# tohinz/multiple-objects-gan

Hardware: AMD Instinct MI355X
Metric: images/sec per G+D train step, 256x256 coco-attngan (higher is better)
Workload: dtype f32

## Files before the change

include/mogan_hip.h:

```cpp
#ifndef MOGAN_HIP_H
#define MOGAN_HIP_H

#include <stddef.h>
#include <stdint.h>

#ifdef __cplusplus
extern "C" {
#endif

typedef struct ihipStream_t* hipStream_t;

#define MOGAN_ERR_SHAPE (-1)
#define MOGAN_ERR_LAUNCH (-2)
#define MOGAN_ERR_WS (-3)

#define MOGAN_ACT_NONE 0
#define MOGAN_ACT_RELU 1
#define MOGAN_ACT_LRELU 2
#define MOGAN_ACT_GLU 3
#define MOGAN_ACT_TANH 4
#define MOGAN_ACT_SIGMOID 5

int mogan_abi_version(void);
int mogan_gemm_set_split_target(int blocks);
int mogan_stream_set_split_target(hipStream_t stream, int blocks);

int mogan_gemm_tune_set(int mode, int M, int N, int K, int nz, int cfg, int split);
int mogan_gemm_tune_clear(void);

int mogan_reserve_streams(int n);

int mogan_gemm_debug_force(int cfg, int split);
int mogan_gemm_group_min_tiles(int tiles);
int mogan_mfma_form(void);

int mogan_prof_enable(int on);
int mogan_prof_collect(double* out, int max_rows);
int mogan_prof_dump(const char* path);

int mogan_conv2d_out_dims(int Hs, int Ws, int KH, int KW, int stride, int ph, int pw, int up, int* OH, int* OW);
int mogan_conv2d_fwd(const float* x, const float* w, float* y, int B, int Cin, int Hs, int Ws, int Cout, int KH,
                     int KW, int stride, int ph, int pw, int up, void* ws, size_t ws_bytes, hipStream_t stream);
int mogan_logits_head_fwd(const float* x, const float* w, const float* bias, float* p, int B, int K, int Cout,
                          hipStream_t stream);
int mogan_logits_head_bwd(const float* dp, const float* p, const float* x, const float* w, float* dx, float* dw, float* db,
                          int B, int K, int Cout, int accumulate, hipStream_t stream);
int mogan_conv2d_lrelu_fwd(const float* x, const float* w, float* z, int B, int Cin, int Hs, int Ws, int Cout, int KH, int KW,
                           int stride, int ph, int pw, float slope, void* ws, size_t ws_bytes, hipStream_t stream);
int mogan_conv2d_affine_fwd(const float* x, const float* w, const float* scale, const float* shift, float* y, int B,
                            int Cin, int Hs, int Ws, int Cout, int KH, int KW, int stride, int ph, int pw, int relu,
                            void* ws, size_t ws_bytes, hipStream_t stream);
int mogan_affine_relu_bwd_out(const float* y, const float* dy, const float* scale, float* dx, int B, int C, int HW,
                              hipStream_t stream);
typedef struct MoganConvFwdArgs {
    const float* x; long long x_bstride; const float* w; const float* scale; const float* shift;
    float* y; long long y_bstride; float* y2; long long y2_bstride; int msplit;
    int B, Cin, Hs, Ws, Cout, KH, KW, stride, ph, pw, relu;
} MoganConvFwdArgs;
typedef struct MoganConvDgradArgs {
    const float* dy; long long dy_bstride; const float* w; float* dx; long long dx_bstride;
    const float* relu_of; long long relu_bstride; int accumulate;
    int B, Cin, Hs, Ws, Cout, KH, KW, stride, ph, pw;
} MoganConvDgradArgs;
int mogan_conv2d_affine_fwd_group(int n, const MoganConvFwdArgs* args, void* ws, size_t ws_bytes, hipStream_t stream);
int mogan_conv2d_dgrad_group(int n, const MoganConvDgradArgs* args, void* ws, size_t ws_bytes, hipStream_t stream);
int mogan_conv2d_affine_fwd_ex(const float* x, long long x_bstride, const float* w, const float* scale, const float* shift,
                               float* y, long long y_bstride, float* y2, long long y2_bstride, int msplit, int B, int Cin,
                               int Hs, int Ws, int Cout, int KH, int KW, int stride, int ph, int pw, int relu, void* ws,
                               size_t ws_bytes, hipStream_t stream);
int mogan_conv2d_fwd_ex(const float* x, long long x_bstride, const float* w, float* y, long long y_bstride,
                        const float* relu_of, long long relu_bstride, int accumulate, int B, int Cin, int Hs, int Ws,
                        int Cout, int KH, int KW, int stride, int ph, int pw, void* ws, size_t ws_bytes, hipStream_t stream);
int mogan_conv2d_dgrad_ex(const float* dy, long long dy_bstride, const float* w, float* dx, long long dx_bstride,
                          const float* relu_of, long long relu_bstride, int accumulate, int B, int Cin, int Hs, int Ws,
                          int Cout, int KH, int KW, int stride, int ph, int pw, void* ws, size_t ws_bytes,
                          hipStream_t stream);
int mogan_conv2d_dgrad(const float* dy, const float* w, float* dx, int B, int Cin, int Hs, int Ws, int Cout, int KH,
                       int KW, int stride, int ph, int pw, int up, void* ws, size_t ws_bytes, hipStream_t stream);
size_t mogan_wino_prep_bytes(int B, int Cin, int Hs, int Ws, int Cout, int KH, int KW, int stride, int ph, int pw, int up, int dgrad);
int mogan_wino_prep_group(int n, const float* const* w, void* const* prep, const int* Cout, const int* Cin, const int* dgrad,
                          hipStream_t stream);
size_t mogan_conv_prep_bytes(int B, int Cin, int Hs, int Ws, int Cout, int KH, int KW, int stride, int ph, int pw, int up, int dgrad);
int mogan_conv_prep_group(int n, const float* const* w, void* const* prep, const int* Cout, const int* Cin, const int* KH,
                          const int* dgrad, hipStream_t stream);
int mogan_conv2d_fwd_wp(const float* x, const float* w, const void* wprep, float* y, int B, int Cin, int Hs, int Ws, int Cout, int KH,
                        int KW, int stride, int ph, int pw, int up, void* ws, size_t ws_bytes, hipStream_t stream);
int mogan_conv2d_dgrad_wp(const float* dy, const float* w, const void* wprep, float* dx, int B, int Cin, int Hs, int Ws, int Cout,
                          int KH, int KW, int stride, int ph, int pw, int up, void* ws, size_t ws_bytes, hipStream_t stream);
int mogan_conv2d_wgrad(const float* dy, const float* x, float* dw, int B, int Cin, int Hs, int Ws, int Cout, int KH,
                       int KW, int stride, int ph, int pw, int up, int accumulate, void* ws, size_t ws_bytes,
                       hipStream_t stream);

int mogan_pk_conv_eligible(int B, int Cin, int Hs, int Ws, int Cout, int KH, int KW, int stride, int ph, int pw, int dgrad);
size_t mogan_pk_weight_bytes(int Cout, int Cin, int KH, int KW, int stride, int dgrad);
int mogan_pk_weight_pack(const float* w, void* wpk, int Cout, int Cin, int KH, int KW, int stride, int ph, int pw, int dgrad,
                         hipStream_t stream);
int mogan_pk_weight_pack_both(const float* w, void* wpk_fwd, void* wpk_dgrad, int Cout, int Cin, int KH, int KW, int stride, int ph,
                              int pw, hipStream_t stream);
int mogan_pk_adam_pack_both(float* p, float* g, float* m, float* v, float* ema, void* wpk_fwd, void* wpk_dgrad, int Cout, int Cin,
                            int KH, int KW, int stride, int ph, int pw, float lr, float beta1, float beta2, float eps, int step,
                            const float* dev_state, int eps_mode, float grad_scale, float ema_decay, int zero_g,
                            hipStream_t stream);
int mogan_conv2d_fwd_pk(const float* x, const void* wpk, float* y, int B, int Cin, int Hs, int Ws, int Cout, int KH, int KW,
                        int stride, int ph, int pw, void* ws, size_t ws_bytes, hipStream_t stream);
int mogan_conv2d_dgrad_pk(const float* dy, const void* wpk, float* dx, int B, int Cin, int Hs, int Ws, int Cout, int KH, int KW,
                          int stride, int ph, int pw, void* ws, size_t ws_bytes, hipStream_t stream);
int mogan_pk_debug_force(int take_all, int cfg, int split);
int mogan_pk_wgrad_eligible(int B, int Cin, int Hs, int Ws, int Cout, int KH, int KW, int stride, int ph, int pw, size_t ws_bytes);
int mogan_conv2d_wgrad_pk(const float* dy, const float* x, float* dw, int B, int Cin, int Hs, int Ws, int Cout, int KH, int KW,
                          int stride, int ph, int pw, int accumulate, void* ws, size_t ws_bytes, hipStream_t stream);

size_t mogan_pk_panel_bytes(int B, int C, int HW);
int mogan_deep_block_eligible(int B, int Cin, int Hs, int Ws, int Cout, int KH, int KW, int stride, int ph, int pw, int act,
                              int groups);
int mogan_deep_conv_bn_act_fwd(const float* x, const void* xpanel, const void* wpk, const float* gamma, const float* beta,
                               float* rmean, float* rvar, float* y, float* stats, float* z, void* zpanel, int B, int Cin, int Hs,
                               int Ws, int Cout, int KH, int KW, int stride, int ph, int pw, float eps, float momentum, int act,
                               float slope, int groups, void* ws, size_t ws_bytes, hipStream_t stream);
int mogan_deep_conv_bn_act_bwd(const float* dz, const float* y, const float* stats, const float* gamma, const float* beta,
                               const void* wpk_dgrad, float* dy, float* dgamma, float* dbeta, int accumulate, float* dx, int B,
                               int Cin, int Hs, int Ws, int Cout, int KH, int KW, int stride, int ph, int pw, int act, float slope,
                               int groups, void* ws, size_t ws_bytes, hipStream_t stream);

typedef struct MoganPkArgs {
    const void* wpk; const void* panel; float* raw;
    int B, M;
    int Cp, CGp, cg0;
    int PH, PW, outH, outW;
    int KH, KW, stride, ph, pw, dgrad;
    int nsplit;
} MoganPkArgs;
#define MOGAN_TAIL_MAXSRC 3
typedef struct MoganTailArgs {
    const float* src[MOGAN_TAIL_MAXSRC]; long long src_bs[MOGAN_TAIL_MAXSRC]; long long src_slab[MOGAN_TAIL_MAXSRC];
    int src_nsplit[MOGAN_TAIL_MAXSRC]; int nsrc;
    const float* add; long long add_bs;
    const float* mask; long long mask_bs;
    const float* scale; const float* shift;
    int relu, box;
    float* dst; long long dst_bs;
    void* panel; int CGp, cg0;
    int B, n, H, W;
} MoganTailArgs;
int mogan_pk_group(int n, MoganPkArgs* args, hipStream_t stream);
int mogan_panel_tail_group(int n, const MoganTailArgs* args, hipStream_t stream);

size_t mogan_upconv3x3_ws_bytes(int Cout, int Cin);
int mogan_upconv3x3_k4(const float* w, float* k4, int Cout, int Cin, hipStream_t stream);
int mogan_upconv3x3_k4_group(int n, const float* const* w, float* const* k4, const int* Cout, const int* Cin, hipStream_t stream);
int mogan_upconv3x3_fwd(const float* x, const float* w, float* y, int B, int Cin, int Hs, int Ws, int Cout, void* ws,
                        size_t ws_bytes, hipStream_t stream);
int mogan_upconv3x3_dgrad(const float* dy, const float* w, float* dx, int B, int Cin, int Hs, int Ws, int Cout, void* ws,
                          size_t ws_bytes, hipStream_t stream);
int mogan_upconv3x3_wgrad(const float* dy, const float* x, float* dw, int B, int Cin, int Hs, int Ws, int Cout,
                          int accumulate, void* ws, size_t ws_bytes, hipStream_t stream);
int mogan_down2_sum(const float* du, float* dx, int planes, int H, int W, hipStream_t stream);

int mogan_bmm(const float* a, const float* b, float* c, int batch, int M, int N, int K, long long sAb, long long sAm,
              long long sAk, long long sBb, long long sBk, long long sBn, long long sCb, long long sCm, long long sCn,
              int accumulate, void* ws, size_t ws_bytes, hipStream_t stream);

size_t mogan_bn_ws_bytes(int B, int C, int HW);
int mogan_bn_stats(const float* x, int B, int C, int HW, float eps, float momentum, float* mean, float* invstd,
                   float* running_mean, float* running_var, void* ws, size_t ws_bytes, hipStream_t stream);
int mogan_bn_act_fwd(const float* x, const float* mean, const float* invstd, const float* gamma, const float* beta,
                     const float* residual, float* y, int B, int C, int HW, int act, float slope, hipStream_t stream);
int mogan_bn_running_update(const float* mean, const float* invstd, float* running_mean, float* running_var, int C, long long n,
                            float eps, float momentum, hipStream_t stream);

int mogan_bn_act_fwd_fused(const float* x, const float* gamma, const float* beta, const float* residual, float* running_mean,
                           float* running_var, float* mean, float* invstd, float* y, int B, int C, int HW, int act, float slope,
                           float eps, float momentum, void* ws, size_t ws_bytes, hipStream_t stream);
int mogan_bn_act_grouped_eligible(int G, int B, int C, int HW);
int mogan_bn_act_grouped_fwd(const float* x, const float* gamma, const float* beta, float* running_mean, float* running_var, float* mean,
                             float* invstd, float* y, int G, int B, int C, int HW, int act, float slope, float eps, float momentum,
                             hipStream_t stream);
int mogan_bn_act_grouped_bwd(const float* x, const float* dy, const float* mean, const float* invstd, const float* gamma, const float* beta,
                             float* dx, float* dgamma, float* dbeta, int G, int B, int C, int HW, int act, float slope, int accumulate,
                             hipStream_t stream);
int mogan_bn_act_bwd(const float* x, const float* dy, const float* mean, const float* invstd, const float* gamma,
                     const float* beta, float* dx, float* dgamma, float* dbeta, int B, int C, int HW, int act,
                     float slope, int accumulate, void* ws, size_t ws_bytes, hipStream_t stream);
int mogan_affine_act_fwd(const float* x, const float* scale, const float* shift, float* y, int B, int C, int HW,
                         int act, float slope, hipStream_t stream);
int mogan_affine_act_bwd(const float* x, const float* dy, const float* scale, const float* shift, float* dx, int B,
                         int C, int HW, int act, float slope, hipStream_t stream);

int mogan_act_fwd(const float* x, float* y, int B, int C, int HW, int act, float slope, hipStream_t stream);
int mogan_act_bwd(const float* x, const float* dy, float* dx, int B, int C, int HW, int act, float slope,
                  hipStream_t stream);
int mogan_bias_add(float* y, const float* bias, int rows, int C, int HW, hipStream_t stream);
int mogan_bias_grad(const float* dy, float* dbias, int rows, int C, int HW, int accumulate, hipStream_t stream);
int mogan_add(const float* a, const float* b, float* y, long long n, hipStream_t stream);
int mogan_group_sum(const float* x, float* y, long long n, int G, hipStream_t stream);
int mogan_group_bcast(const float* dy, float* dx, long long n, int G, hipStream_t stream);
int mogan_scale(const float* a, float alpha, float* y, long long n, hipStream_t stream);

int mogan_softmax_fwd(const float* x, float* y, const int32_t* lens, long long outer, int L, long long inner,
                      float scale, hipStream_t stream);
int mogan_softmax_bwd(const float* y, const float* dy, float* dx, const int32_t* lens, long long outer, int L,
                      long long inner, float scale, hipStream_t stream);

int mogan_stn_fwd(const float* x, const float* theta, float* y, int B, int C, int Hin, int Win, int Hout, int Wout,
                  int align_corners, hipStream_t stream);
int mogan_stn_bwd(const float* dy, const float* theta, float* dx, int B, int C, int Hin, int Win, int Hout,
                  int Wout, int align_corners, hipStream_t stream);
int mogan_stn_fwd_ex(const float* x, const float* theta, float* y, int B, int C, int Hin, int Win, int Hout, int Wout,
                     int align_corners, int xB, int x_plane, int theta_G, hipStream_t stream);
int mogan_stn_bwd_ex(const float* dy, const float* theta, float* dx, int B, int C, int Hin, int Win, int Hout, int Wout,
                     int align_corners, int xB, int x_plane, int theta_G, hipStream_t stream);
#define MOGAN_CAT_MAX 4
int mogan_concat_fwd(const void* const* src, const int* C, const int* rows, const long long* sb, const long long* sg,
                     const int* bcast, int nsrc, float* dst, int N, int HW, hipStream_t stream);
int mogan_concat_bwd(const float* ddst, void* const* dsrc, const int* C, const int* rows, const long long* sb,
                     const long long* sg, const int* bcast, int nsrc, int N, int HW, hipStream_t stream);
int mogan_bbox_to_theta(const float* bbox, float* theta, float* theta_inv, int N, hipStream_t stream);

int mogan_attn_fwd(const float* h, const float* src, const uint8_t* mask, float* wc, float* attn, int B, int idf,
                   int Q, int T, int mask_mode, hipStream_t stream);
int mogan_attn_bwd(const float* src, const float* attn, const float* dwc, const float* dattn, float* dh,
                   float* dscore, int B, int idf, int Q, int T, hipStream_t stream);

int mogan_bce_fwd(const float* p, float target, float weight, float* loss, int n, int accumulate,
                  hipStream_t stream);
int mogan_bce_bwd(const float* p, float target, float weight, const float* gout, float* dp, int n,
                  hipStream_t stream);
int mogan_bce_logits_fwd(const float* x, float target, float weight, float* loss, int n, int accumulate,
                         hipStream_t stream);
int mogan_bce_logits_bwd(const float* x, float target, float weight, const float* gout, float* dx, int n,
                         hipStream_t stream);
int mogan_kl_fwd(const float* mu, const float* logvar, float* loss, int n, hipStream_t stream);
int mogan_kl_bwd(const float* mu, const float* logvar, const float* gout, float* dmu, float* dlogvar, int n,
                 hipStream_t stream);

int mogan_reparam_fwd(const float* mu, const float* logvar, const float* eps, float* c, int n, hipStream_t stream);
int mogan_reparam_bwd(const float* logvar, const float* eps, const float* dc, float* dmu, float* dlogvar, int n,
                      hipStream_t stream);

int mogan_damsm_words_fwd(const float* ctx, const float* words, const int32_t* cap_lens, int B, int Bc, int C, int S, int T,
                          float gamma1, float gamma2, float gamma3, float* sim, float* a1, float* a2, float* wc, float* wt,
                          hipStream_t stream);
int mogan_damsm_words_bwd(const float* ctx, const float* words, const int32_t* cap_lens, const float* a1, const float* a2,
                          const float* wc, const float* dsim, int B, int Bc, int C, int S, int T, float gamma1,
                          float gamma2, float gamma3, float* dwc, float* dscore_t, hipStream_t stream);
int mogan_damsm_ce_fwd(const float* sim, const int64_t* labels, const uint8_t* mask, int R, int Q, float* prow,
                       float* pcol, float* nll, float* out2, hipStream_t stream);
int mogan_damsm_ce_bwd(const float* prow, const float* pcol, const int64_t* labels, const float* g0, const float* g1, int R,
                       int Q, float* dsim, hipStream_t stream);
int mogan_damsm_sent_fwd(const float* cnn, const float* rnn, int B, int Bc, int C, float gamma3, float eps, float* sim,
                         hipStream_t stream);
int mogan_damsm_sent_bwd(const float* cnn, const float* rnn, const float* dsim, int B, int Bc, int C, float gamma3,
                         float eps, float* dcnn, hipStream_t stream);
int mogan_scalar_sum(const float* const* in, const float* weights, int n, float* out, hipStream_t stream);
int mogan_scalar_scale(const float* g, const float* weights, int n, float* const* out, hipStream_t stream);

int mogan_maxpool_fwd(const float* x, float* y, uint8_t* idx, int planes, int H, int W, int k, int s,
                      hipStream_t stream);
int mogan_maxpool_bwd(const uint8_t* idx, const float* dy, float* dx, int planes, int H, int W, int k, int s,
                      hipStream_t stream);
int mogan_avgpool_fwd(const float* x, float* y, int planes, int H, int W, int k, int s, int pad, hipStream_t stream);
int mogan_avgpool_bwd(const float* dy, float* dx, int planes, int H, int W, int k, int s, int pad,
                      hipStream_t stream);
int mogan_maxpool_fwd_ex(const float* x, float* y, long long y_bstride, uint8_t* idx, int B, int C, int H, int W, int k,
                         int s, hipStream_t stream);
int mogan_maxpool_bwd_ex(const uint8_t* idx, const float* dy, long long dy_bstride, float* dx, const float* relu_of,
                         int accumulate, int B, int C, int H, int W, int k, int s, hipStream_t stream);
int mogan_avgpool_bwd_ex(const float* dy, float* dx, const float* relu_of, int accumulate, int planes, int H, int W, int k,
                         int s, int pad, hipStream_t stream);
int mogan_relu_bwd(const float* z, const float* dz, float* dx, long long n, int accumulate, hipStream_t stream);
int mogan_copy_strided(const float* src, long long src_bstride, float* dst, long long dst_bstride, int B, long long n,
                       hipStream_t stream);
int mogan_bilinear_fwd(const float* x, float* y, int planes, int H, int W, int OH, int OW, hipStream_t stream);
int mogan_bilinear_bwd(const float* dy, float* dx, int planes, int H, int W, int OH, int OW, hipStream_t stream);

int mogan_feed_crop_flip(const uint8_t* src, const int32_t* params, uint8_t* q, float* out, int B, int ori, int size,
                         hipStream_t stream);
int mogan_feed_resample(const uint8_t* in, uint8_t* tmp, float* out, const int32_t* bounds, const int32_t* kk, int ksize,
                        int B, int S, int OS, hipStream_t stream);

int mogan_adam_step(float* p, const float* g, float* m, float* v, float* ema, long long n, float lr, float beta1,
                    float beta2, float eps, int step, float* dev_state, int eps_mode, float grad_scale,
                    float ema_decay, hipStream_t stream);
int mogan_adam_prep(float* dev_state, float lr, float beta1, float beta2, int eps_mode, hipStream_t stream);
int mogan_adam_apply(float* p, const float* g, float* m, float* v, float* ema, long long n, float beta1, float beta2, float eps,
                     const float* dev_state, int eps_mode, float grad_scale, float ema_decay, hipStream_t stream);

int mogan_lstm_encoder_fwd(const long long* captions, const int* lens, const float* emb, const float* const* w_ih,
                           const float* const* w_hh, const float* const* b_ih, const float* const* b_hh, const float* h0,
                           const float* c0, float* words, float* sent, int B, int T, int Tmax, int V, int E, int H,
                           hipStream_t stream);

int mogan_lstm_encoder_train_fwd(const long long* captions, const int* lens, const float* emb, const float* const* w_ih,
                                 const float* const* w_hh, const float* const* b_ih, const float* const* b_hh, const float* h0,
                                 const float* c0, const uint8_t* keep_mask, float scale, float* words, float* sent, float* x,
                                 float* gates, float* cells, float* hprev, int B, int T, int Tmax, int V, int E, int H,
                                 hipStream_t stream);
int mogan_lstm_encoder_bwd(const float* dwords, const float* dsent, const int* lens, const float* gates, const float* cells,
                           const float* hprev, const float* c0, const float* const* w_hh, float* dgates, float* dbias, int B,
                           int Tmax, int H, hipStream_t stream);
int mogan_embedding_bwd(const long long* captions, const int* lens, const float* dx, const uint8_t* keep_mask, float scale,
                        float* demb, int B, int T, int Tmax, int V, int E, hipStream_t stream);

int mogan_gru_encoder_fwd(const long long* captions, const int* lens, const float* emb, const float* const* w_ih,
                          const float* const* w_hh, const float* const* b_ih, const float* const* b_hh, const float* h0,
                          float* words, float* sent, int B, int T, int Tmax, int V, int E, int H, hipStream_t stream);
int mogan_gru_encoder_train_fwd(const long long* captions, const int* lens, const float* emb, const float* const* w_ih,
                                const float* const* w_hh, const float* const* b_ih, const float* const* b_hh, const float* h0,
                                const uint8_t* keep_mask, float scale, float* words, float* sent, float* x, float* gates, float* hn,
                                float* hprev, int B, int T, int Tmax, int V, int E, int H, hipStream_t stream);
int mogan_gru_encoder_bwd(const float* dwords, const float* dsent, const int* lens, const float* gates, const float* hn,
                          const float* hprev, const float* const* w_hh, float* dgi, float* dgh, float* dbias_ih, float* dbias_hh,
                          int B, int Tmax, int H, hipStream_t stream);

int mogan_damsm_words_bwd_text(const float* words, const int32_t* cap_lens, const float* wc, const float* dsim, int B, int Bc,
                               int C, int T, float gamma2, float gamma3, float* dwords, hipStream_t stream);
int mogan_damsm_sent_bwd_text(const float* cnn, const float* rnn, const float* dsim, int B, int Bc, int C, float gamma3,
                              float eps, float* drnn, hipStream_t stream);

int mogan_retrieval_rank(const float* code, const float* pos, const float* bank, const int32_t* idx, int Q, int Rn, int C,
                         long long N, float eps, float* score, int32_t* rank, hipStream_t stream);

int mogan_col_mean_f64(const float* x, long long N, int D, double* mean, hipStream_t stream);
int mogan_cov_f64(const float* x, const double* mean, long long N, int D, double* cov, hipStream_t stream);

size_t mogan_poly3_mmd_ws_bytes(int S, int s);
int mogan_poly3_mmd_f64(const float* x, long long Nx, const float* y, long long Ny, int D, const int32_t* ix, const int32_t* iy,
                        int S, int s, double gamma, double coef0, double* sums, void* ws, size_t ws_bytes, hipStream_t stream);

size_t mogan_knn_sqdist_ws_bytes(long long N, int K);
int mogan_knn_sqdist_f64(const float* x, long long N, int D, int K, double* out, void* ws, size_t ws_bytes, hipStream_t stream);
size_t mogan_ball_count_ws_bytes(long long M, long long N, int R);
int mogan_ball_count_f64(const float* q, long long M, const float* p, long long N, int D, const double* r2, int R, int side,
                         int32_t* count, void* ws, size_t ws_bytes, hipStream_t stream);

size_t mogan_knn_cross_ws_bytes(long long M, long long N, int K);
int mogan_knn_cross_f64(const float* q, long long M, const float* p, long long N, int D, int K, double* d2, int32_t* idx, void* ws,
                        size_t ws_bytes, hipStream_t stream);

size_t mogan_knn_label_ws_bytes(long long M, long long N, int K);
int mogan_knn_label_f64(const float* q, const int32_t* qlabel, long long M, const float* p, const int32_t* plabel, long long N, int D,
                        int K, double* d2, int32_t* idx, double* same_d2, int32_t* same_idx, double* other_d2, int32_t* other_idx,
                        void* ws, size_t ws_bytes, hipStream_t stream);

int mogan_pyr_down(const float* x, long long NC, int H, int W, float* out, hipStream_t stream);
int mogan_lap_residual(const float* x, const float* down, long long NC, int H, int W, float* out, hipStream_t stream);
int mogan_swd_gather(const float* level, int N, int C, int H, int W, const int32_t* centres, long long R, float* desc,
                     long long row0, long long rows_total, hipStream_t stream);
size_t mogan_swd_moments_ws_bytes(long long rows, int C);
int mogan_swd_moments_f64(const float* desc, long long rows, int C, double* moments, void* ws, size_t ws_bytes,
                          hipStream_t stream);
int mogan_swd_project(const float* desc, long long rows, int C, const double* moments, const float* dirs, int D, float* out,
                      hipStream_t stream);
int mogan_swd_absdiff_f64(const float* a, const float* b, long long rows, int D, double* out, hipStream_t stream);

int mogan_avg_down2(const float* x, long long NC, int H, int W, float* out, hipStream_t stream);
size_t mogan_ssim_level_ws_bytes(long long P, int C, int S, int n);
int mogan_ssim_level_f64(const float* a, const float* b, long long P, int C, int S, const float* win, int n, double* terms,
                         float* ssim_map, float* cs_map, void* ws, size_t ws_bytes, hipStream_t stream);

int mogan_roi_resize(const float* x, int B, int C, int H, int W, const float* boxes, const int* image_index, long long R,
                     float* y, int OH, int OW, hipStream_t stream);

size_t mogan_radial_power_ws_bytes(int B, int S);
int mogan_radial_power_f64(const float* x, int B, int C, int S, const float* weight, const float* window, const double* twiddle,
                           const int* bins, int n_bins, double* out, void* ws, size_t ws_bytes, hipStream_t stream);

int mogan_box_shift_sums_f64(const float* a, const float* b, long long P, int C, int S, const int* edit, const int* others, int G,
                             double* sums, int* counts, hipStream_t stream);

size_t mogan_softmax_head_ws_bytes(long long n, int C, int S);
int mogan_softmax_head_f64(const float* x, long long n, int D, const float* w, const float* bias, int C, int S, double* row_lse,
                           double* row_h, double* psum, void* ws, size_t ws_bytes, hipStream_t stream);

int mogan_attn_conf_f64(const float* attn, const int* cap_lens, int B, int T, int att, double* conf, hipStream_t stream);
int mogan_attn_sheet_f64(const float* attn, const int* cap_lens, const float* img, const double* table, const int* pick, int P, int B,
                         int T, int att, int vis, int alpha, unsigned char* sheet, double* stats, int* flags, hipStream_t stream);

#ifdef __cplusplus
}
#endif
#endif
```

multiple-objects-gan_amd/csrc/mogan_internal.h:

```cpp
#ifndef MOGAN_INTERNAL_H
#define MOGAN_INTERNAL_H
#include <hip/hip_runtime.h>
#include <stddef.h>
#define MOGAN_HIDDEN __attribute__((visibility("hidden")))

struct MoganConvShape { int B, Cin, Hs, Ws, Cout, KH, KW, stride, ph, pw, up, H, W, OH, OW; };
static inline bool mogan_is_k33(const MoganConvShape& g) { return g.KH == 3 && g.KW == 3 && g.stride == 1 && g.ph == 1 && g.pw == 1; }
static inline bool mogan_is_k44(const MoganConvShape& g) {
    return g.KH == 4 && g.KW == 4 && g.stride == 2 && g.ph == 1 && g.pw == 1 && g.up == 0;
}

MOGAN_HIDDEN int mogan_dconv_fwd_try(const float* x, const float* w, float* y, const MoganConvShape& g, void* ws, size_t ws_bytes,
                                     hipStream_t st, const void* d2prep = nullptr, size_t* d2query = nullptr);
MOGAN_HIDDEN int mogan_dconv_dgrad_try(const float* dy, const float* w, float* dx, const MoganConvShape& g, void* ws,
                                       size_t ws_bytes, hipStream_t st, const void* d2prep = nullptr, size_t* d2query = nullptr);
MOGAN_HIDDEN int mogan_dconv_wgrad_try(const float* dy, const float* x, float* dw, const MoganConvShape& g, int accumulate,
                                       void* ws, size_t ws_bytes, hipStream_t st);
MOGAN_HIDDEN int mogan_dconv2_fwd_try(const float* X, const float* w, int wmode, float* Y, int B, int Cin, int Cout, int H, int W,
                                      int OH, int OW, int KH, int KW, int pt, int pl, int yH, int yW, int ys, int npar,
                                      int accumulate, void* ws, size_t ws_bytes, hipStream_t st, const void* prep = nullptr,
                                      size_t* query = nullptr);
MOGAN_HIDDEN int mogan_smallc_fwd_try(const float* x, const float* w, float* y, const MoganConvShape& g, hipStream_t st);
MOGAN_HIDDEN int mogan_smallc_dgrad_try(const float* dy, const float* w, float* dx, const MoganConvShape& g, hipStream_t st);
MOGAN_HIDDEN int mogan_smallc_wgrad_try(const float* dy, const float* x, float* dw, const MoganConvShape& g, int accumulate,
                                        void* ws, size_t ws_bytes, hipStream_t st);
MOGAN_HIDDEN int mogan_wino_try(const float* in, const float* w, const void* prep, float* out, const MoganConvShape& g, int dgrad,
                                const float* ep_scale, const float* ep_shift, int ep_relu, void* ws, size_t ws_bytes, hipStream_t st);
MOGAN_HIDDEN int mogan_wino_wgrad_try(const float* dy, const float* x, float* dw, const MoganConvShape& g, int accumulate, void* ws,
                                      size_t ws_bytes, hipStream_t st);
MOGAN_HIDDEN void mogan_splitk_reduce_dense(const float* ws, float* out, long long n, int nsplit, int accumulate, hipStream_t st);
MOGAN_HIDDEN int mogan_split_target(hipStream_t st);
MOGAN_HIDDEN int mogan_stem_fwd_try(const float* x, const float* w, float* y, const MoganConvShape& g, float slope, hipStream_t st);
MOGAN_HIDDEN int mogan_dconv2_prep_group(int n, const float* const* w, void* const* prep, const int* Cout, const int* Cin,
                                         const int* dgrad, hipStream_t st);
MOGAN_HIDDEN void mogan_prof_begin(int mode, int cfg, double flops, int M, int N, int K, hipStream_t st);
MOGAN_HIDDEN void mogan_prof_end(int taken, hipStream_t st);
MOGAN_HIDDEN void mogan_prof_relabel(int cfg);
MOGAN_HIDDEN extern int mogan_use_dconv;
#endif
```

multiple-objects-gan_amd/csrc/mogan_pgemm.hip:

```cpp
#include <hip/hip_runtime.h>
#include <stdint.h>
#include <stdlib.h>
#include <algorithm>
#include "../../include/mogan_hip.h"
#include "mogan_internal.h"
#include "mogan_mma.h"
#include "mogan_bn.h"
#include "mogan_adam.h"
#include <math.h>
#include <type_traits>
#ifndef PK_NSET
#define PK_NSET 3
#endif
#define PK_TRIP (PK_NSET == 2 ? 2 : 6)

namespace {

typedef float f32x16 __attribute__((ext_vector_type(16)));

struct PkP {
    const unsigned char* A;
    const unsigned char* P;
    float* C; float* ws;
    int M, N, K;
// ... 454 lines not shown
}
__device__ __forceinline__ void panel_from_lds(const float* L, int NE, unsigned char* P, int C, int c0) {
    const int cg = c0 >> 5, g8 = (c0 & 31) >> 3;
    for (int e = threadIdx.x; e < NE; e += blockDim.x) {
        uint32_t w[3][4];
#pragma unroll
        for (int j = 0; j < 4; ++j) x6_split2(L[(2 * j) * NE + e], L[(2 * j + 1) * NE + e], w[0][j], w[1][j], w[2][j]);
        unsigned char* d = P + ((size_t)e * (C >> 5) + cg) * 192 + g8 * 16;
#pragma unroll
        for (int pl = 0; pl < 3; ++pl) *(uint4*)(d + pl * 64) = make_uint4(w[pl][0], w[pl][1], w[pl][2], w[pl][3]);
    }
}

struct TailP {
    const float* src; int nsplit; long long slab;
    const float* gamma; const float* beta; float* rmean; float* rvar;
    float* y; float* mean; float* invstd; float* z; unsigned char* zpanel;
    int B, C, HW, G; float eps, momentum, slope;
};

template <int ACT, int EPT, int GT>
__global__ __launch_bounds__(256 * GT) void deep_tail_fwd_kernel(const TailP p) {
    extern __shared__ float L[];
    __shared__ float S[GT * 8 * 2];
    const int tid = threadIdx.x & 255, grp = threadIdx.x >> 8, chl = tid >> 5, j = tid & 31;
    const int c0 = blockIdx.x * 8, c = c0 + chl;
    const int NE = p.B * p.HW, b0 = grp * p.B;
    float v[EPT];
    unsigned idx[EPT];
#pragma unroll
    for (int i = 0; i < EPT; ++i) {
        const int e = j + 32 * i;
        const int b = e / p.HW, pos = e - b * p.HW;
        idx[i] = ((unsigned)(b0 + b) * p.C + c) * p.HW + pos;
        v[i] = e < NE ? p.src[idx[i]] : 0.f;
    }
    constexpr int SB = EPT <= 8 ? 4 : (EPT <= 16 ? 2 : 1);
    int sp = 1;
    for (; sp + SB <= p.nsplit; sp += SB) {
        float a[SB][EPT];
#pragma unroll
        for (int u = 0; u < SB; ++u)
#pragma unroll
            for (int i = 0; i < EPT; ++i) a[u][i] = (j + 32 * i) < NE ? p.src[(size_t)(sp + u) * p.slab + idx[i]] : 0.f;
#pragma unroll
        for (int u = 0; u < SB; ++u)
#pragma unroll
            for (int i = 0; i < EPT; ++i) v[i] += a[u][i];
    }
    for (; sp < p.nsplit; ++sp) {
        const float* sl = p.src + (size_t)sp * p.slab;
        float a[EPT];
#pragma unroll
        for (int i = 0; i < EPT; ++i) a[i] = (j + 32 * i) < NE ? sl[idx[i]] : 0.f;
#pragma unroll
        for (int i = 0; i < EPT; ++i) v[i] += a[i];
    }
    double s1 = 0.0, s2 = 0.0;
    const bool wr = p.nsplit > 1 || p.src != p.y;
#pragma unroll
    for (int i = 0; i < EPT; ++i) {
        if (j + 32 * i < NE) {
            if (wr) p.y[idx[i]] = v[i];
            s1 += (double)v[i]; s2 += (double)v[i] * v[i];
        }
    }
    s1 = half_wave_sum(s1); s2 = half_wave_sum(s2);
    const double n = (double)NE;
    float mu, is;
    double var;
    bn_stats_of(s1, s2, n, p.eps, mu, is, var);
    if (j == 0) {
        p.mean[grp * p.C + c] = mu; p.invstd[grp * p.C + c] = is;
        if (GT == 1) {
            bn_running_update(p.rmean, p.rvar, c, mu, var, n, p.momentum);
        } else {
            S[(grp * 8 + chl) * 2] = mu; S[(grp * 8 + chl) * 2 + 1] = (float)bn_unbiased(var, n);
        }
    }
    const BnCoef k = bn_coef(mu, is, p.gamma, p.beta, c);
    const int NT = NE * GT;
#pragma unroll
    for (int i = 0; i < EPT; ++i) {
        const int e = j + 32 * i;
        if (e < NE) {
            const float t = bn_fwd_elem<ACT>(v[i], 0.f, k, k, p.slope);
            p.z[idx[i]] = t;
            if (p.zpanel) L[chl * NT + grp * NE + e] = t;
        }
    }
    if (p.zpanel || GT > 1) __syncthreads();
    if (GT > 1 && grp == 0 && j == 0) {
        float rm = p.rmean ? p.rmean[c] : 0.f, rv = p.rvar ? p.rvar[c] : 0.f;
        for (int g = 0; g < GT; ++g) {
            rm = bn_running_mix(rm, S[(g * 8 + chl) * 2], p.momentum);
            rv = bn_running_mix(rv, S[(g * 8 + chl) * 2 + 1], p.momentum);
        }
        if (p.rmean) p.rmean[c] = rm;
        if (p.rvar) p.rvar[c] = rv;
    }
    if (p.zpanel) panel_from_lds(L, NT, p.zpanel, p.C, c0);
}

struct TailBwdP {
    const float* dz; const float* y; const float* mean; const float* invstd; const float* gamma; const float* beta;
    float* dy; unsigned char* dypanel; float* dgamma; float* dbeta; int accumulate;
    int B, C, HW, G; float slope;
};

template <int ACT, int EPT, int GT>
__global__ __launch_bounds__(256 * GT) void deep_tail_bwd_kernel(const TailBwdP p) {
    extern __shared__ float L[];
    __shared__ float S[GT * 8 * 2];
    const int tid = threadIdx.x & 255, grp = threadIdx.x >> 8, chl = tid >> 5, j = tid & 31;
    const int c0 = blockIdx.x * 8, c = c0 + chl;
    const int NE = p.B * p.HW, b0 = grp * p.B, NT = NE * GT;
    const BnCoef k = bn_coef(p.mean[grp * p.C + c], p.invstd[grp * p.C + c], p.gamma, p.beta, c);
    float g[EPT], xh[EPT];
    double a0 = 0.0, a1 = 0.0;
#pragma unroll
    for (int i = 0; i < EPT; ++i) {
        const int e = j + 32 * i;
        g[i] = 0.f; xh[i] = 0.f;
        if (e < NE) {
            const int b = e / p.HW, pos = e - b * p.HW;
            const size_t idx = ((size_t)(b0 + b) * p.C + c) * p.HW + pos;
            const float xa = p.y[idx];
            float da, dgate;
            act_bwd<ACT>(xa, 0.f, p.dz[idx], k, k, p.slope, da, dgate);
            g[i] = da; xh[i] = bn_xhat(k, xa);
            a0 += da; a1 += (double)da * xh[i];
        }
    }
    a0 = half_wave_sum(a0); a1 = half_wave_sum(a1);
    const float f0 = (float)a0, f1 = (float)a1;
    if (j == 0) {
        if (GT == 1) {
            bn_write_dparam(p.dgamma, p.dbeta, c, f0, f1, p.accumulate);
        } else {
            S[(grp * 8 + chl) * 2] = f0; S[(grp * 8 + chl) * 2 + 1] = f1;
        }
    }
    const float inv_n = 1.f / ((float)p.B * (float)p.HW);
#pragma unroll
    for (int i = 0; i < EPT; ++i) {
        const int e = j + 32 * i;
        if (e < NE) {
            const int b = e / p.HW, pos = e - b * p.HW;
            const float d = bn_dx(k.sc, g[i], xh[i], f0, f1, inv_n);
            p.dy[((size_t)(b0 + b) * p.C + c) * p.HW + pos] = d;
            if (p.dypanel) L[chl * NT + grp * NE + e] = d;
        }
    }
    if (p.dypanel || GT > 1) __syncthreads();
    if (GT > 1 && grp == 0 && j == 0) {
        float db = (p.accumulate && p.dbeta) ? p.dbeta[c] : 0.f, dg = (p.accumulate && p.dgamma) ? p.dgamma[c] : 0.f;
        for (int q = 0; q < GT; ++q) { db += S[(q * 8 + chl) * 2]; dg += S[(q * 8 + chl) * 2 + 1]; }
        if (p.dbeta) p.dbeta[c] = db;
        if (p.dgamma) p.dgamma[c] = dg;
    }
    if (p.dypanel) panel_from_lds(L, NT, p.dypanel, p.C, c0);
}

template <typename K>
static void tail_lds_attr(K kern, size_t lds) {
    if (lds > 60 * 1024) hipFuncSetAttribute((const void*)kern, hipFuncAttributeMaxDynamicSharedMemorySize, 144 * 1024);
}
template <int ACT, int EPT, int GT>
static void launch_tail_fwd_g(const TailP& p, size_t lds, hipStream_t st) {
    static bool attr = false;
    if (!attr && lds > 60 * 1024) { tail_lds_attr(deep_tail_fwd_kernel<ACT, EPT, GT>, lds); attr = true; }
    hipLaunchKernelGGL((deep_tail_fwd_kernel<ACT, EPT, GT>), dim3(p.C / 8), dim3(256 * GT), lds, st, p);
}
template <int ACT, int EPT>
static void launch_tail_fwd_e(const TailP& p, size_t lds, hipStream_t st) {
    if (p.G == 2) launch_tail_fwd_g<ACT, (EPT < 64 ? EPT : 32), 2>(p, lds, st); else launch_tail_fwd_g<ACT, EPT, 1>(p, lds, st);
}
template <int ACT, int EPT, int GT>
static void launch_tail_bwd_g(const TailBwdP& p, size_t lds, hipStream_t st) {
    static bool attr = false;
    if (!attr && lds > 60 * 1024) { tail_lds_attr(deep_tail_bwd_kernel<ACT, EPT, GT>, lds); attr = true; }
    hipLaunchKernelGGL((deep_tail_bwd_kernel<ACT, EPT, GT>), dim3(p.C / 8), dim3(256 * GT), lds, st, p);
}
template <int ACT, int EPT>
static void launch_tail_bwd_e(const TailBwdP& p, size_t lds, hipStream_t st) {
    if (p.G == 2) launch_tail_bwd_g<ACT, (EPT < 64 ? EPT : 32), 2>(p, lds, st); else launch_tail_bwd_g<ACT, EPT, 1>(p, lds, st);
}
template <int ACT>
static int launch_tail_fwd(const TailP& p, hipStream_t st) {
    const int NE = p.B * p.HW;
    const size_t lds = p.zpanel ? (size_t)8 * NE * p.G * sizeof(float) : 0;
    if (NE <= 256) launch_tail_fwd_e<ACT, 8>(p, lds, st);
    else if (NE <= 512) launch_tail_fwd_e<ACT, 16>(p, lds, st);
    else if (NE <= 1024) launch_tail_fwd_e<ACT, 32>(p, lds, st);
    else launch_tail_fwd_e<ACT, 64>(p, lds, st);
    return 0;
}
template <int ACT>
static int launch_tail_bwd(const TailBwdP& p, hipStream_t st) {
    const int NE = p.B * p.HW;
    const size_t lds = p.dypanel ? (size_t)8 * NE * p.G * sizeof(float) : 0;
    if (NE <= 256) launch_tail_bwd_e<ACT, 8>(p, lds, st);
    else if (NE <= 512) launch_tail_bwd_e<ACT, 16>(p, lds, st);
    else if (NE <= 1024) launch_tail_bwd_e<ACT, 32>(p, lds, st);
    else launch_tail_bwd_e<ACT, 64>(p, lds, st);
    return 0;
}
static bool tail_ok(int B, int C, int HW, int act, int G = 1) {
    return B > 0 && HW > 0 && C > 0 && C % 32 == 0 && G >= 1 && G <= 2 && (long long)B * HW * G <= 2048 &&
           (act == MOGAN_ACT_NONE || act == MOGAN_ACT_RELU || act == MOGAN_ACT_LRELU);
}

static inline long long cdiv(long long a, long long b) { return (a + b - 1) / b; }
static inline size_t up256(size_t v) { return (v + 255) & ~(size_t)255; }

static int g_pk_force = 0;

struct PkGeom { int ncls, nkh, nkw, M, Cc, K, Mt, KS; unsigned long long cls_bytes; };

static bool pk_geom(int Cout, int Cin, int KH, int KW, int s, int dgrad, PkGeom& g) {
    if (Cout <= 0 || Cin <= 0 || KH <= 0 || KW <= 0 || s <= 0) return false;
    if (!dgrad) {
        if (Cin % 32) return false;
        g.ncls = 1; g.nkh = KH; g.nkw = KW; g.M = Cout; g.Cc = Cin;
    } else {
        if (Cout % 32 || KH % s || KW % s) return false;
        g.ncls = s * s; g.nkh = KH / s; g.nkw = KW / s; g.M = Cin; g.Cc = Cout;
    }
    if (KH * KW > 25) return false;
    g.K = g.nkh * g.nkw * g.Cc;
    g.Mt = (int)cdiv(g.M, 32); g.KS = g.K / 16;
    g.cls_bytes = (unsigned long long)g.Mt * g.KS * 3072ull;
    return g.cls_bytes < (1ull << 32);
}

struct PkCfg { int tm, tn; };
static const PkCfg kPk[] = {{1, 2}, {1, 4}, {2, 2}};
enum { NPK = 3 };
static int g_pk_cfg = -1, g_pk_split = 0;
#ifndef PK_OCC12
#define PK_OCC12 3
#endif
#ifndef PK_G64_OCC
#define PK_G64_OCC 2
#endif
static int g_pk_group_tile = -1;
static inline int a_prof_mode(int dgrad) { return dgrad ? 11 : 10; }

template <int TM, int TN, int OCC>
static void launch_pk(unsigned blocks, hipStream_t st, const PkP& p) {
    hipLaunchKernelGGL((pgemm_kernel<TM, TN, OCC>), dim3(blocks), dim3(256), 0, st, p);
}

static int run_pk(PkP& p, void* ws, size_t ws_bytes, int prof_mode, hipStream_t st, bool keep_slabs = false) {
    int best = 0; double bestw = 1e300;
    for (int c = 0; c < NPK; ++c) {
        const int bm = 128 * kPk[c].tm, bn = 32 * kPk[c].tn;
        double w = (double)cdiv(p.M, bm) * bm * (double)cdiv(p.N, bn) * bn;
        w *= c == 0 ? 1.0 : 1.15;
        if (w < bestw * 0.999) { bestw = w; best = c; }
    }
    if (g_pk_cfg >= 0) best = g_pk_cfg;
    const int bm = 128 * kPk[best].tm, bn = 32 * kPk[best].tn;
    p.gx = (int)cdiv(p.N, bn); p.gy = (int)cdiv(p.M, bm);
    const long long tiles = (long long)p.gx * p.gy * p.ncls;
    const long long c_numel = (long long)p.slab;
    int nsplit = 1;
    const int target = mogan_split_target(st);
    if (tiles < target && p.ntile >= 8) {
        nsplit = (int)cdiv(target, tiles);
        nsplit = std::min(nsplit, p.ntile / 4);
        if (nsplit < 1) nsplit = 1;
    }
    if (g_pk_split > 0) nsplit = std::min(g_pk_split, p.ntile);
    if (nsplit > 1) {
        const long long fit = ws ? (long long)(ws_bytes / (sizeof(float) * (size_t)c_numel)) : 0;
        if (fit < 2) nsplit = 1; else nsplit = (int)std::min<long long>(nsplit, fit);
    }
    p.kt_per = (int)cdiv(cdiv(p.ntile, nsplit), PK_TRIP) * PK_TRIP;
    p.nsplit = (int)cdiv(p.ntile, p.kt_per);
    p.ws = (float*)ws;
    const long long blocks = tiles * p.nsplit;
    if (blocks <= 0 || blocks > 0x7fffffff) return MOGAN_ERR_SHAPE;
    const double flops = 2.0 * (double)p.M * (double)p.N * p.ncls * (double)p.K;
    mogan_prof_begin(prof_mode, best, flops, p.M, p.N * p.ncls, p.K, st);
    switch (best) {
        case 1: launch_pk<1, 4, 2>((unsigned)blocks, st, p); break;
        case 2: launch_pk<2, 2, 2>((unsigned)blocks, st, p); break;
        default: launch_pk<1, 2, PK_OCC12>((unsigned)blocks, st, p); break;
    }
    mogan_prof_end(1, st);
    if (p.nsplit > 1 && !keep_slabs) mogan_splitk_reduce_dense((const float*)ws, p.C, c_numel, p.nsplit, p.accumulate, st);
    return hipGetLastError() == hipSuccess ? 0 : MOGAN_ERR_LAUNCH;
}

static int apack(const float* x, unsigned char* P, int B, int C, int HW, hipStream_t st) {
    const long long Q = (long long)B * HW;
    hipLaunchKernelGGL(apack_kernel, dim3((unsigned)cdiv(Q, 64), (unsigned)(C / 32)), dim3(256), 0, st, x, P, B, C, HW);
    return 0;
}

}

extern "C" {

int mogan_pk_debug_force(int take_all, int cfg, int split) {
    g_pk_force = take_all; g_pk_cfg = (cfg >= 0 && cfg < NPK) ? cfg : -1; g_pk_split = split > 0 ? split : 0;
    return 0;
}

int mogan_pk_conv_eligible(int B, int Cin, int Hs, int Ws, int Cout, int KH, int KW, int stride, int ph, int pw, int dgrad) {
    PkGeom g;
    if (B <= 0 || Hs <= 0 || Ws <= 0 || !pk_geom(Cout, Cin, KH, KW, stride, dgrad, g)) return 0;
    const int OH = (Hs + 2 * ph - KH) / stride + 1, OW = (Ws + 2 * pw - KW) / stride + 1;
    if (OH <= 0 || OW <= 0) return 0;
    if (dgrad && (Hs % stride || Ws % stride)) return 0;
    const long long pix = dgrad ? (long long)B * OH * OW : (long long)B * Hs * Ws;
    if (pix * g.Cc * 6 >= (1ll << 32)) return 0;
    if (g_pk_force) return 1;
    const int rows_hw = dgrad ? (Hs / stride) * (Ws / stride) : OH * OW;
    return rows_hw <= 64 && g.K >= 1024 && g.M >= 128;
}

size_t mogan_pk_weight_bytes(int Cout, int Cin, int KH, int KW, int stride, int dgrad) {
    PkGeom g;
    if (!pk_geom(Cout, Cin, KH, KW, stride, dgrad, g)) return 0;
    return (size_t)g.cls_bytes * g.ncls;
}

int mogan_pk_weight_pack(const float* w, void* wpk, int Cout, int Cin, int KH, int KW, int stride, int ph, int pw, int dgrad,
                         hipStream_t stream) {
    PkGeom g;
    if (!w || !wpk || !pk_geom(Cout, Cin, KH, KW, stride, dgrad, g)) return MOGAN_ERR_SHAPE;
    WpackP p{};
    p.w = w; p.A = (unsigned char*)wpk; p.Cout = Cout; p.Cin = Cin; p.KH = KH; p.KW = KW; p.s = dgrad ? stride : 1;
    p.ph = ph; p.pw = pw; p.dgrad = dgrad; p.M = g.M; p.Cc = g.Cc; p.Mt = g.Mt; p.KS = g.KS; p.cls_stride = g.cls_bytes;
    if (g.Cc % 16) return MOGAN_ERR_SHAPE;
    const size_t lds = (size_t)KH * KW * 32 * 17 * sizeof(float);
    hipLaunchKernelGGL(wpack_kernel, dim3((unsigned)g.Mt, (unsigned)(g.Cc / 16)), dim3(256), lds, stream, p);
    return hipGetLastError() == hipSuccess ? 0 : MOGAN_ERR_LAUNCH;
}

}

namespace {
static int pk_fwd_from_panel(const void* panel, const void* wpk, float* y, int B, int Cin, int Hs, int Ws, int Cout, int KH, int KW,
                             int stride, int ph, int pw, void* ws, size_t ws_bytes, hipStream_t stream, bool keep_slabs,
                             int* nsplit_out, int accumulate = 0, int prof_mode = 7) {
    PkGeom g;
    if (!pk_geom(Cout, Cin, KH, KW, stride, 0, g) || B <= 0) return MOGAN_ERR_SHAPE;
    const int OH = (Hs + 2 * ph - KH) / stride + 1, OW = (Ws + 2 * pw - KW) / stride + 1;
    if (OH <= 0 || OW <= 0) return MOGAN_ERR_SHAPE;
    const size_t pbytes = (size_t)B * Hs * Ws * Cin * 6;
    if (pbytes >= (1ull << 32) || (long long)B * Cout * OH * OW >= (1ll << 31)) return MOGAN_ERR_SHAPE;
    PkP p{};
    p.A = (const unsigned char*)wpk; p.P = (const unsigned char*)panel; p.C = y;
    p.M = Cout; p.N = B * OH * OW; p.K = g.K; p.Mt = g.Mt; p.KS = g.KS; p.a_cls_stride = g.cls_bytes;
    p.a_bytes = (unsigned)g.cls_bytes; p.p_bytes = (unsigned)pbytes; p.ntile = g.K / 32; p.slab = (long long)B * Cout * OH * OW;
    p.accumulate = accumulate; p.dgrad = 0; p.ncls = 1; p.Cc = Cin; p.CG = Cin / 32; p.CGp = Cin / 32; p.cg0 = 0; p.PH = Hs; p.PW = Ws; p.RH = OH; p.RW = OW;
    p.s = stride; p.ph = ph; p.pw = pw; p.nkw = KW; p.outH = OH; p.outW = OW;
    const int rc = run_pk(p, ws, ws_bytes, prof_mode, stream, keep_slabs);
    if (nsplit_out) *nsplit_out = p.nsplit;
    return rc;
}
static int pk_dgrad_from_panel(const void* panel, const void* wpk, float* dx, int B, int Cin, int Hs, int Ws, int Cout, int KH,
                               int KW, int stride, int ph, int pw, void* ws, size_t ws_bytes, hipStream_t stream) {
    PkGeom g;
    if (!pk_geom(Cout, Cin, KH, KW, stride, 1, g) || B <= 0 || Hs % stride || Ws % stride) return MOGAN_ERR_SHAPE;
    const int OH = (Hs + 2 * ph - KH) / stride + 1, OW = (Ws + 2 * pw - KW) / stride + 1;
    if (OH <= 0 || OW <= 0) return MOGAN_ERR_SHAPE;
    const size_t pbytes = (size_t)B * OH * OW * Cout * 6;
    if (pbytes >= (1ull << 32) || (long long)B * Cin * Hs * Ws >= (1ll << 31)) return MOGAN_ERR_SHAPE;
    PkP p{};
    p.A = (const unsigned char*)wpk; p.P = (const unsigned char*)panel; p.C = dx;
    p.M = Cin; p.N = B * (Hs / stride) * (Ws / stride); p.K = g.K; p.Mt = g.Mt; p.KS = g.KS; p.a_cls_stride = g.cls_bytes;
    p.a_bytes = (unsigned)g.cls_bytes; p.p_bytes = (unsigned)pbytes; p.ntile = g.K / 32; p.slab = (long long)B * Cin * Hs * Ws;
    p.accumulate = 0; p.dgrad = 1; p.ncls = stride * stride; p.Cc = Cout; p.CG = Cout / 32; p.CGp = Cout / 32; p.cg0 = 0; p.PH = OH; p.PW = OW;
    p.RH = Hs / stride; p.RW = Ws / stride; p.s = stride; p.ph = ph; p.pw = pw; p.nkw = g.nkw; p.outH = Hs; p.outW = Ws;
    return run_pk(p, ws, ws_bytes, 8, stream);
}
}

static bool deep_geom_ok(int B, int Cin, int Hs, int Ws, int Cout, int KH, int KW, int stride, int OH, int OW, int dgrad) {
    PkGeom g;
    if (!pk_geom(Cout, Cin, KH, KW, stride, dgrad, g) || B <= 0 || Hs <= 0 || Ws <= 0 || OH <= 0 || OW <= 0) return false;
    if (dgrad && (Hs % stride || Ws % stride)) return false;
    const unsigned long long pbytes = dgrad ? (unsigned long long)B * OH * OW * Cout * 6 : (unsigned long long)B * Hs * Ws * Cin * 6;
    const long long out = dgrad ? (long long)B * Cin * Hs * Ws : (long long)B * Cout * OH * OW;
    return pbytes < (1ull << 32) && out < (1ll << 31);
}

extern "C" {

int mogan_conv2d_fwd_pk(const float* x, const void* wpk, float* y, int B, int Cin, int Hs, int Ws, int Cout, int KH, int KW,
                        int stride, int ph, int pw, void* ws, size_t ws_bytes, hipStream_t stream) {
    if (B <= 0 || Cin <= 0 || Cin % 32 || Hs <= 0 || Ws <= 0) return MOGAN_ERR_SHAPE;
    const size_t pbytes = (size_t)B * Hs * Ws * Cin * 6;
    if (!ws || ws_bytes < up256(pbytes)) return MOGAN_ERR_WS;
    apack(x, (unsigned char*)ws, B, Cin, Hs * Ws, stream);
    return pk_fwd_from_panel(ws, wpk, y, B, Cin, Hs, Ws, Cout, KH, KW, stride, ph, pw, (char*)ws + up256(pbytes),
                             ws_bytes - up256(pbytes), stream, false, nullptr);
}

int mogan_conv2d_dgrad_pk(const float* dy, const void* wpk, float* dx, int B, int Cin, int Hs, int Ws, int Cout, int KH, int KW,
                          int stride, int ph, int pw, void* ws, size_t ws_bytes, hipStream_t stream) {
    if (B <= 0 || Cout <= 0 || Cout % 32 || stride <= 0) return MOGAN_ERR_SHAPE;
    const int OH = (Hs + 2 * ph - KH) / stride + 1, OW = (Ws + 2 * pw - KW) / stride + 1;
    if (OH <= 0 || OW <= 0) return MOGAN_ERR_SHAPE;
    const size_t pbytes = (size_t)B * OH * OW * Cout * 6;
    if (!ws || ws_bytes < up256(pbytes)) return MOGAN_ERR_WS;
    apack(dy, (unsigned char*)ws, B, Cout, OH * OW, stream);
    return pk_dgrad_from_panel(ws, wpk, dx, B, Cin, Hs, Ws, Cout, KH, KW, stride, ph, pw, (char*)ws + up256(pbytes),
                               ws_bytes - up256(pbytes), stream);
}

int mogan_pk_weight_pack_both(const float* w, void* wpk_fwd, void* wpk_dgrad, int Cout, int Cin, int KH, int KW, int stride, int ph,
                              int pw, hipStream_t stream) {
    PkGeom gf, gd;
    if (!w || !wpk_fwd || !wpk_dgrad || !pk_geom(Cout, Cin, KH, KW, stride, 0, gf) || !pk_geom(Cout, Cin, KH, KW, stride, 1, gd))
        return MOGAN_ERR_SHAPE;
    if (Cin % 32) return MOGAN_ERR_SHAPE;
    Wpack2P p{};
    p.w = w; p.Af = (unsigned char*)wpk_fwd; p.Ad = (unsigned char*)wpk_dgrad; p.Cout = Cout; p.Cin = Cin; p.KW = KW; p.s = stride;
    p.ph = ph; p.pw = pw; p.KSf = gf.KS; p.KSd = gd.KS; p.cls_stride = gd.cls_bytes;
    const dim3 grid((unsigned)cdiv(Cout, 32), (unsigned)(Cin / 16));
    switch (KH * KW) {
        case 16: hipLaunchKernelGGL(wpack2_kernel<16>, grid, dim3(256), 0, stream, p); break;
        case 9: hipLaunchKernelGGL(wpack2_kernel<9>, grid, dim3(256), 0, stream, p); break;
        case 1: hipLaunchKernelGGL(wpack2_kernel<1>, grid, dim3(256), 0, stream, p); break;
        default: {
            int rc = mogan_pk_weight_pack(w, wpk_fwd, Cout, Cin, KH, KW, stride, ph, pw, 0, stream);
            return rc ? rc : mogan_pk_weight_pack(w, wpk_dgrad, Cout, Cin, KH, KW, stride, ph, pw, 1, stream);
        }
    }
    return hipGetLastError() == hipSuccess ? 0 : MOGAN_ERR_LAUNCH;
}

int mogan_pk_adam_pack_both(float* p, float* g, float* m, float* v, float* ema, void* wpk_fwd, void* wpk_dgrad, int Cout, int Cin,
                            int KH, int KW, int stride, int ph, int pw, float lr, float beta1, float beta2, float eps, int step,
                            const float* dev_state, int eps_mode, float grad_scale, float ema_decay, int zero_g,
                            hipStream_t stream) {
    PkGeom gf, gd;
    if (!p || !g || !m || !v || !wpk_fwd || !wpk_dgrad || (!dev_state && step < 1)) return MOGAN_ERR_SHAPE;
    if ((((uintptr_t)p | (uintptr_t)g | (uintptr_t)m | (uintptr_t)v | (uintptr_t)ema | (uintptr_t)wpk_fwd | (uintptr_t)wpk_dgrad) & 15) != 0)
        return MOGAN_ERR_SHAPE;
    if (!pk_geom(Cout, Cin, KH, KW, stride, 0, gf) || !pk_geom(Cout, Cin, KH, KW, stride, 1, gd)) return MOGAN_ERR_SHAPE;
    if (Cin % 32 || Cout % 32) return MOGAN_ERR_SHAPE;
    const int taps = KH * KW;
    if (taps != 16 && taps != 9 && taps != 1) return MOGAN_ERR_SHAPE;
    Wpack2AdamP a{};
    a.pk.w = p; a.pk.Af = (unsigned char*)wpk_fwd; a.pk.Ad = (unsigned char*)wpk_dgrad; a.pk.Cout = Cout; a.pk.Cin = Cin;
    a.pk.KW = KW; a.pk.s = stride; a.pk.ph = ph; a.pk.pw = pw; a.pk.KSf = gf.KS; a.pk.KSd = gd.KS; a.pk.cls_stride = gd.cls_bytes;
    a.p = p; a.g = g; a.m = m; a.v = v; a.ema = ema; a.dev_state = dev_state;
    a.beta1 = beta1; a.beta2 = beta2; a.eps = eps; a.eps_mode = eps_mode; a.gscale = grad_scale; a.ema_decay = ema_decay;
    a.zero_g = zero_g ? 1 : 0;
    if (!dev_state) {
        const double bc1 = 1.0 - pow((double)beta1, (double)step), bc2 = 1.0 - pow((double)beta2, (double)step);
        a.step_size = eps_mode == 0 ? (float)(lr / bc1) : (float)(lr * sqrt(bc2) / bc1);
        a.inv_sqrt_bc2 = (float)(1.0 / sqrt(bc2));
    }
    const dim3 grid((unsigned)(Cout / 32), (unsigned)(Cin / 16));
#define MOGAN_ADAM_PACK(T)                                                                                          \
    if (ema) hipLaunchKernelGGL((wpack2_adam_kernel<T, true>), grid, dim3(256), 0, stream, a);                      \
    else hipLaunchKernelGGL((wpack2_adam_kernel<T, false>), grid, dim3(256), 0, stream, a)
    switch (taps) {
        case 16: MOGAN_ADAM_PACK(16); break;
        case 9: MOGAN_ADAM_PACK(9); break;
        default: MOGAN_ADAM_PACK(1); break;
    }
#undef MOGAN_ADAM_PACK
    return hipGetLastError() == hipSuccess ? 0 : MOGAN_ERR_LAUNCH;
}

static bool wgrad_pk_sizes(int B, int Cin, int Hs, int Ws, int Cout, int KH, int KW, int stride, int ph, int pw, int& OH, int& OW,
                           int& Kpad, long long& R, size_t& abytes, size_t& pbytes) {
    if (B <= 0 || Cin <= 0 || Cout <= 0 || Hs <= 0 || Ws <= 0 || KH <= 0 || KW <= 0 || stride <= 0) return false;
    OH = (Hs + 2 * ph - KH) / stride + 1; OW = (Ws + 2 * pw - KW) / stride + 1;
    if (OH <= 0 || OW <= 0) return false;
    const long long npix = (long long)B * OH * OW;
    if (npix > (1 << 20)) return false;
    Kpad = (int)((npix + 31) / 32 * 32);
    R = (long long)Cin * KH * KW;
    abytes = up256((size_t)((Cout + 31) / 32) * 32 * Kpad * 6);
    pbytes = up256((size_t)R * Kpad * 6);
    return pbytes < (1ull << 32) && (long long)Cout * R < (1ll << 31);
}

int mogan_pk_wgrad_eligible(int B, int Cin, int Hs, int Ws, int Cout, int KH, int KW, int stride, int ph, int pw, size_t ws_bytes) {
    int OH, OW, Kpad; long long R; size_t ab, pb;
    if (!wgrad_pk_sizes(B, Cin, Hs, Ws, Cout, KH, KW, stride, ph, pw, OH, OW, Kpad, R, ab, pb)) return 0;
    if (ab + pb > ws_bytes) return 0;
    if (g_pk_force) return 1;
    return OH * OW <= 64 && Kpad >= 512 && (long long)Cout * R >= (16ll << 20);
}

int mogan_conv2d_wgrad_pk(const float* dy, const float* x, float* dw, int B, int Cin, int Hs, int Ws, int Cout, int KH, int KW,
                          int stride, int ph, int pw, int accumulate, void* ws, size_t ws_bytes, hipStream_t stream) {
    int OH, OW, Kpad; long long R; size_t ab, pb;
    if (!dy || !x || !dw || !wgrad_pk_sizes(B, Cin, Hs, Ws, Cout, KH, KW, stride, ph, pw, OH, OW, Kpad, R, ab, pb)) return MOGAN_ERR_SHAPE;
    if (!ws || ab + pb > ws_bytes) return MOGAN_ERR_WS;
    unsigned char* A = (unsigned char*)ws;
    unsigned char* P = A + ab;
    const int Mt = (Cout + 31) / 32, KS = Kpad / 16, npix = B * OH * OW;
    hipLaunchKernelGGL(dypack_kernel, dim3((unsigned)cdiv((long long)Mt * KS * 64, 256)), dim3(256), 0, stream, dy, A, Cout, OH * OW,
                       npix, KS);
    XtP q{};
    q.x = x; q.P = P; q.Cin = Cin; q.Hs = Hs; q.Ws = Ws; q.KH = KH; q.KW = KW; q.s = stride; q.ph = ph; q.pw = pw; q.OH = OH; q.OW = OW;
    q.Npix = npix; q.KG = Kpad / 32; q.total = R * (Kpad / 8);
    hipLaunchKernelGGL(xtpack_kernel, dim3((unsigned)cdiv(q.total, 256)), dim3(256), 0, stream, q);
    return pk_fwd_from_panel(P, A, dw, 1, Kpad, (int)R, 1, Cout, 1, 1, 1, 0, 0, (char*)ws + ab + pb, ws_bytes - ab - pb, stream, false,
                             nullptr, accumulate, 9);
}

int mogan_pk_group(int n, MoganPkArgs* args, hipStream_t stream) {
    constexpr int env_tile = -1;
    g_pk_group_tile = env_tile;
    if (n <= 0 || n > PK_MAXG || !args) return MOGAN_ERR_SHAPE;
    PkGroup g{};
    g.n = n;
    long long end = 0; double flops = 0;
    double w128 = 0, w64 = 0;
    for (int i = 0; i < n; ++i) {
        const double N = (double)args[i].B * args[i].outH * args[i].outW, K = (double)args[i].KH * args[i].KW * args[i].Cp;
        w128 += (double)cdiv(args[i].M, 128) * 128 * (double)cdiv((long long)N, 64) * 64 * K;
        w64 += (double)cdiv(args[i].M, 64) * 64 * (double)cdiv((long long)N, 128) * 128 * K;
    }
    (void)w64; (void)w128;
    const int tile64 = g_pk_group_tile > 0 ? 1 : 0;
    const int bm = tile64 ? 64 : 128, bn = tile64 ? 128 : 64;
    for (int i = 0; i < n; ++i) {
        const MoganPkArgs& a = args[i];
        if (!a.wpk || !a.panel || !a.raw || a.B <= 0 || a.M <= 0 || a.Cp <= 0 || a.Cp % 32 || a.cg0 < 0 || a.cg0 + a.Cp / 32 > a.CGp ||
            a.KH <= 0 || a.KW <= 0 || a.KH * a.KW > 25 || a.stride <= 0 || (a.dgrad && a.stride != 1) || a.PH <= 0 || a.PW <= 0 ||
            a.outH <= 0 || a.outW <= 0 || a.nsplit <= 0)
            return MOGAN_ERR_SHAPE;
        const size_t pbytes = (size_t)a.B * a.PH * a.PW * a.CGp * 192;
        const long long slab = (long long)a.B * a.M * a.outH * a.outW;
        PkP& p = g.p[i];
        p.A = (const unsigned char*)a.wpk; p.P = (const unsigned char*)a.panel; p.C = a.raw; p.ws = a.raw;
        p.M = a.M; p.N = a.B * a.outH * a.outW; p.K = a.KH * a.KW * a.Cp; p.Mt = (int)cdiv(p.M, 32); p.KS = p.K / 16;
        const unsigned long long abytes = (unsigned long long)p.Mt * p.KS * 3072ull;
        if (pbytes >= (1ull << 32) || abytes >= (1ull << 32) || slab >= (1ll << 31)) return MOGAN_ERR_SHAPE;
        p.a_cls_stride = abytes; p.a_bytes = (unsigned)abytes; p.p_bytes = (unsigned)pbytes; p.ntile = p.K / 32; p.slab = slab;
        p.accumulate = 0; p.dgrad = a.dgrad; p.ncls = 1; p.Cc = a.Cp; p.CG = a.Cp / 32; p.CGp = a.CGp; p.cg0 = a.cg0;
        p.PH = a.PH; p.PW = a.PW; p.RH = a.outH; p.RW = a.outW; p.s = a.stride; p.ph = a.ph; p.pw = a.pw; p.nkw = a.KW;
        p.outH = a.outH; p.outW = a.outW;
        p.gx = (int)cdiv(p.N, bn); p.gy = (int)cdiv(p.M, bm);
        p.kt_per = (int)cdiv(cdiv(p.ntile, std::min(a.nsplit, p.ntile)), PK_TRIP) * PK_TRIP;
        while (cdiv(p.ntile, p.kt_per) > a.nsplit) p.kt_per += PK_TRIP;
        p.nsplit = (int)cdiv(p.ntile, p.kt_per);
        args[i].nsplit = p.nsplit;
        end += (long long)p.gx * p.gy * p.nsplit;
        if (end > 0x7fffffff) return MOGAN_ERR_SHAPE;
        g.end[i] = (unsigned)end;
        flops += 2.0 * (double)p.M * (double)p.N * (double)p.K;
    }
    mogan_prof_begin(a_prof_mode(args[0].dgrad), tile64, flops, g.p[0].M, g.p[0].N, g.p[0].K, stream);
    if (tile64) hipLaunchKernelGGL((pgemm_group_kernel<1, 2, PK_G64_OCC, 2>), dim3((unsigned)end), dim3(256), 0, stream, g);
    else hipLaunchKernelGGL((pgemm_group_kernel<1, 2, 3, 4>), dim3((unsigned)end), dim3(256), 0, stream, g);
    mogan_prof_end(1, stream);
    return hipGetLastError() == hipSuccess ? 0 : MOGAN_ERR_LAUNCH;
}

size_t mogan_pk_panel_bytes(int B, int C, int HW) { return (B > 0 && C > 0 && HW > 0) ? (size_t)B * HW * C * 6 : 0; }

int mogan_deep_block_eligible(int B, int Cin, int Hs, int Ws, int Cout, int KH, int KW, int stride, int ph, int pw, int act,
                              int groups) {
    if (groups < 1 || B <= 0 || B % groups) return 0;
    if (!mogan_pk_conv_eligible(B, Cin, Hs, Ws, Cout, KH, KW, stride, ph, pw, 0)) return 0;
    if (!mogan_pk_conv_eligible(B, Cin, Hs, Ws, Cout, KH, KW, stride, ph, pw, 1)) return 0;
    const int OH = (Hs + 2 * ph - KH) / stride + 1, OW = (Ws + 2 * pw - KW) / stride + 1;
    return tail_ok(B / groups, Cout, OH * OW, act, groups) ? 1 : 0;
}

int mogan_deep_conv_bn_act_fwd(const float* x, const void* xpanel, const void* wpk, const float* gamma, const float* beta,
                               float* rmean, float* rvar, float* y, float* stats, float* z, void* zpanel, int B, int Cin, int Hs,
                               int Ws, int Cout, int KH, int KW, int stride, int ph, int pw, float eps, float momentum, int act,
                               float slope, int groups, void* ws, size_t ws_bytes, hipStream_t stream) {
    if (B <= 0 || groups < 1 || B % groups || Cin <= 0 || Cin % 32 || Hs <= 0 || Ws <= 0 || stride <= 0) return MOGAN_ERR_SHAPE;
    const int OH = (Hs + 2 * ph - KH) / stride + 1, OW = (Ws + 2 * pw - KW) / stride + 1;
    if (OH <= 0 || OW <= 0 || !tail_ok(B / groups, Cout, OH * OW, act, groups) || !gamma || !beta || !y || !stats || !z || !wpk ||
        (!x && !xpanel) || !deep_geom_ok(B, Cin, Hs, Ws, Cout, KH, KW, stride, OH, OW, 0))
        return MOGAN_ERR_SHAPE;
    char* w0 = (char*)ws; size_t wn = ws_bytes;
    if (!xpanel) {
        const size_t pbytes = up256((size_t)B * Hs * Ws * Cin * 6);
        if (!ws || ws_bytes < pbytes) return MOGAN_ERR_WS;
        apack(x, (unsigned char*)ws, B, Cin, Hs * Ws, stream);
        xpanel = ws; w0 += pbytes; wn -= pbytes;
    }
    int nsplit = 1;
    int rc = pk_fwd_from_panel(xpanel, wpk, y, B, Cin, Hs, Ws, Cout, KH, KW, stride, ph, pw, w0, wn, stream, true, &nsplit);
    if (rc) return rc;
    TailP t{};
    t.src = nsplit > 1 ? (const float*)w0 : y; t.nsplit = nsplit; t.slab = (long long)B * Cout * OH * OW;
    t.gamma = gamma; t.beta = beta; t.rmean = rmean; t.rvar = rvar; t.y = y; t.mean = stats; t.invstd = stats + (size_t)groups * Cout;
    t.z = z; t.zpanel = (unsigned char*)zpanel; t.B = B / groups; t.G = groups; t.C = Cout; t.HW = OH * OW; t.eps = eps;
    t.momentum = momentum; t.slope = slope;
    if (act == MOGAN_ACT_LRELU) launch_tail_fwd<MOGAN_ACT_LRELU>(t, stream);
    else if (act == MOGAN_ACT_RELU) launch_tail_fwd<MOGAN_ACT_RELU>(t, stream);
    else launch_tail_fwd<MOGAN_ACT_NONE>(t, stream);
    return hipGetLastError() == hipSuccess ? 0 : MOGAN_ERR_LAUNCH;
}

int mogan_deep_conv_bn_act_bwd(const float* dz, const float* y, const float* stats, const float* gamma, const float* beta,
                               const void* wpk_dgrad, float* dy, float* dgamma, float* dbeta, int accumulate, float* dx, int B,
                               int Cin, int Hs, int Ws, int Cout, int KH, int KW, int stride, int ph, int pw, int act, float slope,
                               int groups, void* ws, size_t ws_bytes, hipStream_t stream) {
    if (B <= 0 || stride <= 0 || groups < 1 || B % groups || Cin % 32 || KH <= 0 || KW <= 0 || KH * KW > 25) return MOGAN_ERR_SHAPE;
    const int OH = (Hs + 2 * ph - KH) / stride + 1, OW = (Ws + 2 * pw - KW) / stride + 1;
    if (OH <= 0 || OW <= 0 || !tail_ok(B / groups, Cout, OH * OW, act, groups) || !dz || !y || !stats || !gamma || !beta || !dy)
        return MOGAN_ERR_SHAPE;
    const size_t pbytes = up256((size_t)B * OH * OW * Cout * 6);
    const bool want_dx = dx != nullptr;
    if (want_dx && !deep_geom_ok(B, Cin, Hs, Ws, Cout, KH, KW, stride, OH, OW, 1)) return MOGAN_ERR_SHAPE;
    if (want_dx && (!ws || ws_bytes < pbytes || !wpk_dgrad)) return MOGAN_ERR_WS;
    TailBwdP t{};
    t.dz = dz; t.y = y; t.mean = stats; t.invstd = stats + (size_t)groups * Cout; t.gamma = gamma; t.beta = beta; t.dy = dy;
    t.dypanel = want_dx ? (unsigned char*)ws : nullptr; t.dgamma = dgamma; t.dbeta = dbeta; t.accumulate = accumulate;
    t.B = B / groups; t.G = groups; t.C = Cout; t.HW = OH * OW; t.slope = slope;
    if (act == MOGAN_ACT_LRELU) launch_tail_bwd<MOGAN_ACT_LRELU>(t, stream);
    else if (act == MOGAN_ACT_RELU) launch_tail_bwd<MOGAN_ACT_RELU>(t, stream);
    else launch_tail_bwd<MOGAN_ACT_NONE>(t, stream);
    if (!want_dx) return hipGetLastError() == hipSuccess ? 0 : MOGAN_ERR_LAUNCH;
    return pk_dgrad_from_panel(ws, wpk_dgrad, dx, B, Cin, Hs, Ws, Cout, KH, KW, stride, ph, pw, (char*)ws + pbytes,
                               ws_bytes - pbytes, stream);
}

}
```

multiple-objects-gan_amd/hip/lib.py:

```python
import contextlib
import ctypes
import os

import torch

_HERE = os.path.dirname(os.path.dirname(os.path.abspath(__file__)))
LIB_PATH = os.environ.get("MOGAN_LIB") or os.path.join(_HERE, "libmogan_hip.so")

P, I, F, L, Z, D = ctypes.c_void_p, ctypes.c_int, ctypes.c_float, ctypes.c_longlong, ctypes.c_size_t, ctypes.c_double

SIGNATURES = {
    "mogan_abi_version": [],
    "mogan_gemm_set_split_target": [I],
    "mogan_stream_set_split_target": [P, I],
    "mogan_gemm_debug_force": [I, I],
    "mogan_gemm_group_min_tiles": [I],
    "mogan_mfma_form": [],
    "mogan_gemm_tune_set": [I, I, I, I, I, I, I],
    "mogan_gemm_tune_clear": [],
    "mogan_reserve_streams": [ctypes.c_int],
    "mogan_prof_enable": [I],
    "mogan_prof_collect": [P, I],
    "mogan_prof_dump": [ctypes.c_char_p],
    "mogan_conv2d_out_dims": [I, I, I, I, I, I, I, I, P, P],
    "mogan_conv2d_fwd": [P, P, P] + [I] * 11 + [P, Z, P],
    "mogan_logits_head_fwd": [P, P, P, P, I, I, I, P],
    "mogan_logits_head_bwd": [P, P, P, P, P, P, P, I, I, I, I, P],
    "mogan_conv2d_lrelu_fwd": [P, P, P] + [I] * 10 + [F, P, Z, P],
    "mogan_conv2d_affine_fwd": [P, P, P, P, P] + [I] * 11 + [P, Z, P],
    "mogan_affine_relu_bwd_out": [P, P, P, P, I, I, I, P],
    "mogan_conv2d_dgrad": [P, P, P] + [I] * 11 + [P, Z, P],
    "mogan_conv2d_wgrad": [P, P, P] + [I] * 12 + [P, Z, P],
    "mogan_wino_prep_bytes": [I] * 12,
    "mogan_wino_prep_group": [I, P, P, P, P, P, P],
    "mogan_conv_prep_bytes": [I] * 12,
    "mogan_conv_prep_group": [I, P, P, P, P, P, P, P],
    "mogan_conv2d_fwd_wp": [P, P, P, P] + [I] * 11 + [P, Z, P],
    "mogan_conv2d_dgrad_wp": [P, P, P, P] + [I] * 11 + [P, Z, P],
    "mogan_pk_conv_eligible": [I] * 11,
    "mogan_pk_weight_bytes": [I] * 6,
    "mogan_pk_weight_pack": [P, P] + [I] * 8 + [P],
    "mogan_pk_weight_pack_both": [P, P, P] + [I] * 7 + [P],
    "mogan_pk_adam_pack_both": [P] * 7 + [I] * 7 + [F, F, F, F, I, P, I, F, F, I, P],
    "mogan_conv2d_fwd_pk": [P, P, P] + [I] * 10 + [P, Z, P],
    "mogan_conv2d_dgrad_pk": [P, P, P] + [I] * 10 + [P, Z, P],
    "mogan_pk_debug_force": [I, I, I],
    "mogan_pk_wgrad_eligible": [I] * 10 + [Z],
    "mogan_conv2d_wgrad_pk": [P, P, P] + [I] * 11 + [P, Z, P],
    "mogan_pk_panel_bytes": [I, I, I],
    "mogan_deep_block_eligible": [I] * 12,
    "mogan_deep_conv_bn_act_fwd": [P] * 11 + [I] * 10 + [F, F, I, F, I, P, Z, P],
    "mogan_deep_conv_bn_act_bwd": [P] * 9 + [I, P] + [I] * 10 + [I, F, I, P, Z, P],
    "mogan_upconv3x3_ws_bytes": [I, I],
    "mogan_upconv3x3_fwd": [P, P, P, I, I, I, I, I, P, Z, P],
    "mogan_lstm_encoder_fwd": [P] * 11 + [I] * 6 + [P],
    "mogan_upconv3x3_k4": [P, P, I, I, P],
    "mogan_upconv3x3_k4_group": [I, P, P, P, P, P],
    "mogan_upconv3x3_dgrad": [P, P, P, I, I, I, I, I, P, Z, P],
    "mogan_upconv3x3_wgrad": [P, P, P, I, I, I, I, I, I, P, Z, P],
    "mogan_down2_sum": [P, P, I, I, I, P],
    "mogan_bmm": [P, P, P, I, I, I, I] + [L] * 9 + [I, P, Z, P],
    "mogan_bn_ws_bytes": [I, I, I],
    "mogan_bn_stats": [P, I, I, I, F, F, P, P, P, P, P, Z, P],
    "mogan_bn_running_update": [P, P, P, P, I, L, F, F, P],
    "mogan_bn_act_fwd": [P, P, P, P, P, P, P, I, I, I, I, F, P],
    "mogan_bn_act_grouped_eligible": [I, I, I, I],
    "mogan_bn_act_grouped_fwd": [P] * 8 + [I] * 5 + [F, F, F, P],
    "mogan_bn_act_grouped_bwd": [P] * 9 + [I] * 5 + [F, I, P],
    "mogan_bn_act_fwd_fused": [P, P, P, P, P, P, P, P, P, I, I, I, I, F, F, F, P, Z, P],
    "mogan_bn_act_bwd": [P, P, P, P, P, P, P, P, P, I, I, I, I, F, I, P, Z, P],
    "mogan_affine_act_fwd": [P, P, P, P, I, I, I, I, F, P],
    "mogan_affine_act_bwd": [P, P, P, P, P, I, I, I, I, F, P],
    "mogan_act_fwd": [P, P, I, I, I, I, F, P],
    "mogan_act_bwd": [P, P, P, I, I, I, I, F, P],
    "mogan_bias_add": [P, P, I, I, I, P],
    "mogan_bias_grad": [P, P, I, I, I, I, P],
    "mogan_add": [P, P, P, L, P],
    "mogan_group_sum": [P, P, L, I, P],
    "mogan_group_bcast": [P, P, L, I, P],
    "mogan_scale": [P, F, P, L, P],
    "mogan_softmax_fwd": [P, P, P, L, I, L, F, P],
    "mogan_softmax_bwd": [P, P, P, P, L, I, L, F, P],
    "mogan_stn_fwd": [P, P, P, I, I, I, I, I, I, I, P],
    "mogan_stn_bwd": [P, P, P, I, I, I, I, I, I, I, P],
    "mogan_stn_fwd_ex": [P, P, P, I, I, I, I, I, I, I, I, I, I, P],
    "mogan_stn_bwd_ex": [P, P, P, I, I, I, I, I, I, I, I, I, I, P],
    "mogan_concat_fwd": [P, P, P, P, P, P, I, P, I, I, P],
    "mogan_concat_bwd": [P, P, P, P, P, P, P, I, I, I, P],
    "mogan_bbox_to_theta": [P, P, P, I, P],
    "mogan_attn_fwd": [P, P, P, P, P, I, I, I, I, I, P],
    "mogan_attn_bwd": [P, P, P, P, P, P, I, I, I, I, P],
    "mogan_bce_fwd": [P, F, F, P, I, I, P],
    "mogan_bce_bwd": [P, F, F, P, P, I, P],
    "mogan_bce_logits_fwd": [P, F, F, P, I, I, P],
    "mogan_bce_logits_bwd": [P, F, F, P, P, I, P],
    "mogan_kl_fwd": [P, P, P, I, P],
    "mogan_kl_bwd": [P, P, P, P, P, I, P],
    "mogan_reparam_fwd": [P, P, P, P, I, P],
    "mogan_reparam_bwd": [P, P, P, P, P, I, P],
    "mogan_maxpool_fwd": [P, P, P, I, I, I, I, I, P],
    "mogan_maxpool_bwd": [P, P, P, I, I, I, I, I, P],
    "mogan_avgpool_fwd": [P, P, I, I, I, I, I, I, P],
    "mogan_avgpool_bwd": [P, P, I, I, I, I, I, I, P],
    "mogan_bilinear_fwd": [P, P, I, I, I, I, I, P],
    "mogan_bilinear_bwd": [P, P, I, I, I, I, I, P],
    "mogan_adam_step": [P, P, P, P, P, L, F, F, F, F, I, P, I, F, F, P],
    "mogan_adam_prep": [P, F, F, F, I, P],
    "mogan_adam_apply": [P, P, P, P, P, L, F, F, F, P, I, F, F, P],
    "mogan_conv2d_affine_fwd_ex": [P, L, P, P, P, P, L, P, L, I] + [I] * 11 + [P, Z, P],
    "mogan_conv2d_fwd_ex": [P, L, P, P, L, P, L, I] + [I] * 10 + [P, Z, P],
    "mogan_conv2d_dgrad_ex": [P, L, P, P, L, P, L, I] + [I] * 10 + [P, Z, P],
    "mogan_conv2d_affine_fwd_group": [I, P, P, Z, P],
    "mogan_conv2d_dgrad_group": [I, P, P, Z, P],
    "mogan_pk_group": [I, P, P],
    "mogan_panel_tail_group": [I, P, P],
    "mogan_maxpool_fwd_ex": [P, P, L, P, I, I, I, I, I, I, P],
    "mogan_maxpool_bwd_ex": [P, P, L, P, P, I, I, I, I, I, I, I, P],
    "mogan_avgpool_bwd_ex": [P, P, P, I, I, I, I, I, I, I, P],
    "mogan_copy_strided": [P, L, P, L, I, L, P],
    "mogan_relu_bwd": [P, P, P, L, I, P],
    "mogan_feed_crop_flip": [P, P, P, P, I, I, I, P],
    "mogan_feed_resample": [P, P, P, P, P, I, I, I, I, P],
    "mogan_damsm_words_fwd": [P, P, P, I, I, I, I, I, F, F, F, P, P, P, P, P, P],
    "mogan_damsm_words_bwd": [P, P, P, P, P, P, P, I, I, I, I, I, F, F, F, P, P, P],
    "mogan_damsm_ce_fwd": [P, P, P, I, I, P, P, P, P, P],
    "mogan_damsm_ce_bwd": [P, P, P, P, P, I, I, P, P],
    "mogan_damsm_sent_fwd": [P, P, I, I, I, F, F, P, P],
    "mogan_damsm_sent_bwd": [P, P, P, I, I, I, F, F, P, P],
    "mogan_damsm_words_bwd_text": [P, P, P, P, I, I, I, I, F, F, P, P],
    "mogan_damsm_sent_bwd_text": [P, P, P, I, I, I, F, F, P, P],
    "mogan_lstm_encoder_train_fwd": [P] * 10 + [F] + [P] * 6 + [I] * 6 + [P],
    "mogan_lstm_encoder_bwd": [P] * 10 + [I] * 3 + [P],
    "mogan_embedding_bwd": [P, P, P, P, F, P, I, I, I, I, I, P],
    "mogan_gru_encoder_fwd": [P] * 10 + [I] * 6 + [P],
    "mogan_gru_encoder_train_fwd": [P] * 9 + [F] + [P] * 6 + [I] * 6 + [P],
    "mogan_gru_encoder_bwd": [P] * 11 + [I] * 3 + [P],
    "mogan_retrieval_rank": [P, P, P, P, I, I, I, L, F, P, P, P],
    "mogan_col_mean_f64": [P, L, I, P, P],
    "mogan_cov_f64": [P, P, L, I, P, P],
    "mogan_poly3_mmd_ws_bytes": [I, I],
    "mogan_poly3_mmd_f64": [P, L, P, L, I, P, P, I, I, D, D, P, P, Z, P],
    "mogan_knn_sqdist_ws_bytes": [L, I],
    "mogan_knn_sqdist_f64": [P, L, I, I, P, P, Z, P],
    "mogan_ball_count_ws_bytes": [L, L, I],
    "mogan_ball_count_f64": [P, L, P, L, I, P, I, I, P, P, Z, P],
    "mogan_knn_cross_ws_bytes": [L, L, I],
    "mogan_knn_cross_f64": [P, L, P, L, I, I, P, P, P, Z, P],
    "mogan_knn_label_ws_bytes": [L, L, I],
    "mogan_knn_label_f64": [P, P, L, P, P, L, I, I, P, P, P, P, P, P, P, Z, P],
    "mogan_pyr_down": [P, L, I, I, P, P],
    "mogan_lap_residual": [P, P, L, I, I, P, P],
    "mogan_swd_gather": [P, I, I, I, I, P, L, P, L, L, P],
    "mogan_swd_moments_ws_bytes": [L, I],
    "mogan_swd_moments_f64": [P, L, I, P, P, Z, P],
    "mogan_swd_project": [P, L, I, P, P, I, P, P],
    "mogan_swd_absdiff_f64": [P, P, L, I, P, P],
    "mogan_avg_down2": [P, L, I, I, P, P],
    "mogan_ssim_level_ws_bytes": [L, I, I, I],
    "mogan_ssim_level_f64": [P, P, L, I, I, P, I, P, P, P, P, Z, P],
    "mogan_roi_resize": [P, I, I, I, I, P, P, L, P, I, I, P],
    "mogan_radial_power_ws_bytes": [I, I],
    "mogan_radial_power_f64": [P, I, I, I, P, P, P, P, I, P, P, Z, P],
    "mogan_box_shift_sums_f64": [P, P, L, I, I, P, P, I, P, P, P],
    "mogan_softmax_head_ws_bytes": [L, I, I],
    "mogan_softmax_head_f64": [P, L, I, P, P, I, I, P, P, P, P, Z, P],
    "mogan_attn_conf_f64": [P, P, I, I, I, P, P],
    "mogan_attn_sheet_f64": [P, P, P, P, P, I, I, I, I, I, I, P, P, P, P],
    "mogan_scalar_sum": [P, P, I, P, P],
    "mogan_scalar_scale": [P, P, I, P, P],
}


class ConvFwdArgs(ctypes.Structure):
    _fields_ = [("x", P), ("x_bstride", L), ("w", P), ("scale", P), ("shift", P), ("y", P), ("y_bstride", L), ("y2", P),
                ("y2_bstride", L), ("msplit", I)] + [(k, I) for k in ("B", "Cin", "Hs", "Ws", "Cout", "KH", "KW", "stride",
                                                                      "ph", "pw", "relu")]


class ConvDgradArgs(ctypes.Structure):
    _fields_ = [("dy", P), ("dy_bstride", L), ("w", P), ("dx", P), ("dx_bstride", L), ("relu_of", P), ("relu_bstride", L),
                ("accumulate", I)] + [(k, I) for k in ("B", "Cin", "Hs", "Ws", "Cout", "KH", "KW", "stride", "ph", "pw")]


class PkArgs(ctypes.Structure):
    _fields_ = [("wpk", P), ("panel", P), ("raw", P)] + [(k, I) for k in ("B", "M", "Cp", "CGp", "cg0", "PH", "PW", "outH", "outW",
                                                                       "KH", "KW", "stride", "ph", "pw", "dgrad", "nsplit")]


class TailArgs(ctypes.Structure):
    _fields_ = [("src", P * 3), ("src_bs", L * 3), ("src_slab", L * 3), ("src_nsplit", I * 3), ("nsrc", I), ("add", P), ("add_bs", L),
                ("mask", P), ("mask_bs", L), ("scale", P), ("shift", P), ("relu", I), ("box", I), ("dst", P), ("dst_bs", L),
                ("panel", P), ("CGp", I), ("cg0", I), ("B", I), ("n", I), ("H", I), ("W", I)]


_RESTYPE = {"mogan_bn_ws_bytes": Z, "mogan_upconv3x3_ws_bytes": Z, "mogan_pk_weight_bytes": Z, "mogan_pk_panel_bytes": Z,
            "mogan_wino_prep_bytes": Z, "mogan_conv_prep_bytes": Z, "mogan_poly3_mmd_ws_bytes": Z,
            "mogan_knn_sqdist_ws_bytes": Z, "mogan_ball_count_ws_bytes": Z, "mogan_swd_moments_ws_bytes": Z,
            "mogan_ssim_level_ws_bytes": Z, "mogan_knn_cross_ws_bytes": Z, "mogan_radial_power_ws_bytes": Z,
            "mogan_knn_label_ws_bytes": Z, "mogan_softmax_head_ws_bytes": Z}
_ERRORS = {-1: "MOGAN_ERR_SHAPE", -2: "MOGAN_ERR_LAUNCH", -3: "MOGAN_ERR_WS"}

_lib = None
_ws = {}
WORKSPACE_BYTES = int(os.environ.get("MOGAN_WS_MB", "256")) << 20


class MoganHipError(RuntimeError):
    pass


def load():
    global _lib
    if _lib is None:
        if not os.path.isfile(LIB_PATH):
            raise MoganHipError(
                "libmogan_hip.so is not built (%s). Run `python __graft_entry__.py` / "
                "`python multiple-objects-gan_amd/build.py`; there is no CPU fallback." % LIB_PATH)
        lib = ctypes.CDLL(LIB_PATH)
        for name, args in SIGNATURES.items():
            fn = getattr(lib, name)
            fn.argtypes = args
            fn.restype = _RESTYPE.get(name, I)
        _lib = lib
        _register_tuned(lib)
    return _lib


TUNED_CSV = os.path.join(os.path.dirname(os.path.abspath(__file__)), "tuned_gemm_gfx950.csv")


def _register_tuned(lib):
    if os.environ.get("MOGAN_TUNED", "1") == "0" or not os.path.isfile(TUNED_CSV):
        return 0
    n = 0
    with open(TUNED_CSV) as f:
        for line in f:
            if line.startswith("#") or line.startswith("mode") or not line.strip():
                continue
            v = [int(x) for x in line.split(",")[:7]]
            if lib.mogan_gemm_tune_set(*v) == 0:
                n += 1
    return n


_raw_stream = getattr(torch._C, "_cuda_getCurrentRawStream", None)


_reserved = []


def hw_queue_defaults():
    return (os.environ.get("MOGAN_HW_QUEUES", "4"), 0)


def configure_hw_queues():
    os.environ.setdefault("GPU_MAX_HW_QUEUES", hw_queue_defaults()[0])


def reserve_hw_queues(n=None):
    if n is None:
        n = int(hw_queue_defaults()[1])
    if _reserved or n <= 0:
        return
    got = load().mogan_reserve_streams(int(n))
    if got < n:
        raise RuntimeError("mogan_reserve_streams(%d) -> %d" % (n, got))
    _reserved.append(got)


def stream_ptr():
    if _raw_stream is not None:
        return _raw_stream(torch.cuda.current_device())
    return torch.cuda.current_stream().cuda_stream


_capturing = getattr(torch._C, "_cuda_isCurrentStreamCapturing", None) or torch.cuda.is_current_stream_capturing
_cap_epoch = [0, False]


def workspace(device):
    if device.type != "cuda":
        raise MoganHipError("mogan_hip ops need tensors on the GPU (got device %s): there is no CPU "
                            "path in the product" % device)
    idx = device.index if device.index is not None else torch.cuda.current_device()
    handle = _raw_stream(idx) if _raw_stream is not None else torch.cuda.current_stream(device).cuda_stream
    if _capturing():
        if not _cap_epoch[1]:
            _cap_epoch[0] += 1
            _cap_epoch[1] = True
        key = (idx, handle, _cap_epoch[0])
    else:
        _cap_epoch[1] = False
        key = (idx, handle)
    buf = _ws.get(key)
    if buf is None:
        buf = torch.empty(WORKSPACE_BYTES, dtype=torch.uint8, device=device)
        _ws[key] = buf
    return buf.data_ptr(), buf.numel()


def ptr(t):
    if t is None:
        return None
    if not t.is_cuda:
        raise MoganHipError("mogan_hip ops need tensors on the GPU (got a %s tensor): "
                            "there is no CPU path in the product" % t.device)
    return t.data_ptr()


def call(name, *args):
    rc = getattr(load(), name)(*args)
    if rc != 0:
        raise MoganHipError("%s failed: %s" % (name, _ERRORS.get(rc, rc)))


def bn_ws_bytes(B, C, HW):
    return int(load().mogan_bn_ws_bytes(B, C, HW))


@contextlib.contextmanager
def capture_guard():
    import gc
    gc.collect()
    was = gc.isenabled()
    gc.disable()
    try:
        yield
    finally:
        if was:
            gc.enable()
```

multiple-objects-gan_amd/hip/ops.py:

```python
import contextlib
import ctypes
import os

import torch

from . import lib
from .lib import call, ptr, stream_ptr, workspace

ACT_NONE, ACT_RELU, ACT_LRELU, ACT_GLU, ACT_TANH, ACT_SIGMOID = 0, 1, 2, 3, 4, 5

ACT_TRACE = None


BN_DEFER = None


def bn_apply_deferred(pending):
    for mean, invstd, n, rm, rv, eps, momentum in pending:
        if rm is not None or rv is not None:
            call("mogan_bn_running_update", ptr(mean), ptr(invstd), ptr(rm), ptr(rv), mean.numel(), int(n), float(eps),
                 float(momentum), stream_ptr())
    del pending[:]


TRACE_GROUPS = 1


def _trace(act, y, groups=1):
    if groups <= 1:
        ACT_TRACE.append((act, y))
        return
    n = y.shape[0] // groups
    for g in range(groups):
        ACT_TRACE.append((act, y[g * n:(g + 1) * n], g) if TRACE_GROUPS > 1 else (act, y[g * n:(g + 1) * n]))


DIRECT_GRAD = True


GRAD_HOOKS = []


def _grad_hit(g, stream=None):
    if GRAD_HOOKS:
        p = g.data_ptr()
        for lo, hi, cb in GRAD_HOOKS:
            if lo <= p < hi:
                cb(p, stream)
                break


def _grad_buf(param):
    if not DIRECT_GRAD or param is None:
        return None
    g = getattr(param, "grad", None)
    if g is None or not g.is_contiguous() or g.dtype != torch.float32 or g.shape != param.shape:
        return None
    return g


WGRAD_SIDE_STREAM = False
CAPTURE_WGRAD_OK = set()
_WGRAD_ENV = os.environ.get("MOGAN_WGRAD_STREAM", "1") != "0"
_wgrad_streams = {}


class _WgradFrame:
    __slots__ = ("used", "keep", "parked")

    def __init__(self):
        self.used, self.keep, self.parked = [], [], []


_wgrad_frames = [_WgradFrame()]


MERGE_WGRAD = os.environ.get("MOGAN_MERGE_WGRAD", "1") != "0"
_wgrad_pending = {}
MERGE_WGRAD_CAPTURED = True
_wgrad_ctx_depth = 0
_MERGE_K = 2048
_MERGE_W = 1 << 21


FUSE_ADAM_PACK = os.environ.get("MOGAN_FUSE_ADAM_PACK", "1") != "0"
WGRAD_OVERWRITE = os.environ.get("MOGAN_WGRAD_OVERWRITE", "1") != "0"
_OVERWRITE = {}


def overwrite_register(g, round_cell):
    if g.data_ptr() in _OVERWRITE:
        return False
    _OVERWRITE[g.data_ptr()] = [round_cell, round_cell[0]]
    return True


def overwrite_drop(ptrs):
    for p in ptrs:
        _OVERWRITE.pop(p, None)
    del ptrs[:]


def overwrite_stale(g):
    rec = _OVERWRITE.get(g.data_ptr())
    return rec is not None and rec[1] != rec[0][0]


def _first_of_round(g):
    rec = _OVERWRITE.get(g.data_ptr()) if _OVERWRITE else None
    if rec is None:
        return False
    first = rec[1] != rec[0][0]
    rec[1] = rec[0][0]
    return first


def _wgrad_launch(dy, x, w_shape, geom, g):
    stride, ph, pw, up = geom
    acc = not _first_of_round(g)
    if WGRAD_SIDE_STREAM:
        cur, side = _wgrad_stream()
        side.wait_stream(cur)
        with torch.cuda.stream(side):
            conv2d_wgrad(dy, x, w_shape, stride, ph, pw, up, out=g, accumulate=acc)
        fr = _wgrad_frames[-1]
        if side not in fr.used:
            fr.used.append(side)
        fr.keep.append((dy, x))
        _grad_hit(g, side)
    else:
        conv2d_wgrad(dy, x, w_shape, stride, ph, pw, up, out=g, accumulate=acc)
        _grad_hit(g)


def _wgrad_accumulate(dy, x, w, geom, g):
    K = dy.shape[0] * dy.shape[2] * dy.shape[3]
    if not (MERGE_WGRAD and _wgrad_ctx_depth > 0 and K <= _MERGE_K and w.numel() >= _MERGE_W) \
            or (torch.cuda.is_current_stream_capturing() and not MERGE_WGRAD_CAPTURED):
        _wgrad_launch(dy, x, w.shape, geom, g)
        return
    cur = torch.cuda.current_stream()
    key = (g.data_ptr(), cur.cuda_stream)
    prev = _wgrad_pending.pop(key, None)
    if prev is None:
        _wgrad_pending[key] = (dy, x, tuple(w.shape), geom, g, cur)
        _wgrad_frames[-1].parked.append(key)
        return
    pdy, px, _, pgeom = prev[:4]
    if pgeom == geom and pdy.shape[1:] == dy.shape[1:] and px.shape[1:] == x.shape[1:]:
        _wgrad_launch(_cat_batch(pdy, dy), _cat_batch(px, x), w.shape, geom, g)
    else:
        _wgrad_launch(pdy, px, w.shape, pgeom, g)
        _wgrad_launch(dy, x, w.shape, geom, g)


def _cat_batch(a, b):
    a, b = _c(a), _c(b)
    if a.shape[1:] != b.shape[1:]:
        raise lib.MoganHipError("_cat_batch: %r and %r differ behind the batch axis" % (tuple(a.shape), tuple(b.shape)))
    per = a[0].numel()
    out = torch.empty((a.shape[0] + b.shape[0],) + tuple(a.shape[1:]), dtype=torch.float32, device=a.device)
    arrs = _cat_arrays([(a.shape[0], 1, 0, 0, 0), (b.shape[0], 1, 0, 0, 0)], [a.data_ptr(), b.data_ptr()])
    call("mogan_concat_fwd", *arrs, 2, ptr(out), 1, per, stream_ptr())
    return out


class SplitBatchFn(torch.autograd.Function):

    @staticmethod
    def forward(ctx, x, B):
        ctx.B, ctx.shape = B, tuple(x.shape)
        return x[:B], x[B:]

    @staticmethod
    def backward(ctx, da, db):
        B, shape = ctx.B, ctx.shape
        if da is None:
            da = torch.zeros((B,) + shape[1:], dtype=torch.float32, device=db.device)
        if db is None:
            db = torch.zeros((shape[0] - B,) + shape[1:], dtype=torch.float32, device=da.device)
        return _cat_batch(da, db), None


def split_batch(x, B):
    return SplitBatchFn.apply(_c(x), int(B))


def _wgrad_flush():
    cur = torch.cuda.current_stream()
    fr = _wgrad_frames[-1]
    keys, fr.parked = fr.parked, []
    if len(_wgrad_frames) == 1:
        keys = list(_wgrad_pending)
    capturing = torch.cuda.is_current_stream_capturing()
    for key in keys:
        item = _wgrad_pending.pop(key, None)
        if item is None:
            continue
        dy, x, w_shape, geom, g, st = item
        if st.cuda_stream == cur.cuda_stream:
            _wgrad_launch(dy, x, w_shape, geom, g)
        else:
            with torch.cuda.stream(st):
                _wgrad_launch(dy, x, w_shape, geom, g)
            if not capturing:
                cur.wait_stream(st)


@contextlib.contextmanager
def wgrad_overlap():
    global WGRAD_SIDE_STREAM, _wgrad_ctx_depth
    ok = _WGRAD_ENV
    if ok and torch.cuda.is_current_stream_capturing():
        ok = torch.cuda.current_stream().cuda_stream in CAPTURE_WGRAD_OK
    prev, WGRAD_SIDE_STREAM = WGRAD_SIDE_STREAM, ok
    _wgrad_ctx_depth += 1
    _wgrad_frames.append(_WgradFrame())
    try:
        yield
    finally:
        try:
            _wgrad_flush()
        finally:
            _wgrad_ctx_depth -= 1
            WGRAD_SIDE_STREAM = prev
            join_wgrad()
            _wgrad_frames.pop()


def _wgrad_stream():
    cur = torch.cuda.current_stream()
    side = _wgrad_streams.get(cur.cuda_stream)
    if side is None:
        side = _wgrad_streams[cur.cuda_stream] = torch.cuda.Stream()
    return cur, side


def precreate_wgrad_stream(stream):
    if stream.cuda_stream not in _wgrad_streams:
        _wgrad_streams[stream.cuda_stream] = torch.cuda.Stream()
    return _wgrad_streams[stream.cuda_stream]


def join_wgrad():
    fr = _wgrad_frames[-1]
    if not _wgrad_streams:
        del fr.keep[:]
        return
    cur = torch.cuda.current_stream()
    side = _wgrad_streams.get(cur.cuda_stream)
    if side is not None:
        cur.wait_stream(side)
    capturing = torch.cuda.is_current_stream_capturing()
    for s_ in fr.used:
        if s_ is not side and not capturing:
            cur.wait_stream(s_)
    del fr.used[:]
    del fr.keep[:]


def _c(t):
    if t.dtype != torch.float32:
        t = t.float()
    return t if t.is_contiguous() else t.contiguous()


def conv_out_hw(Hs, Ws, KH, KW, stride, ph, pw, up):
    H, W = Hs << up, Ws << up
    return (H + 2 * ph - KH) // stride + 1, (W + 2 * pw - KW) // stride + 1


UPCONV4 = True


def _is_upconv(w_shape, stride, ph, pw, up):
    return UPCONV4 and bool(up) and stride == 1 and ph == 1 and pw == 1 and w_shape[2] == 3 and w_shape[3] == 3


PK_ENABLED = True
PK_STATS = {"fwd": 0, "dgrad": 0, "wgrad": 0, "packs": 0}
PK_WGRAD = True
_pk_wgrad_elig = {}
_PK_GLOBAL = [0]


def invalidate_all_packs():
    _PK_GLOBAL[0] += 1


class WeightImage:
    __slots__ = ("buf", "version", "epoch", "event", "stream", "captured", "geom")

    def __init__(self, buf, geom=None):
        self.buf, self.geom = buf, geom
        self.version = self.epoch = -1
        self.event = self.stream = None
        self.captured = False

    def invalidate(self):
        self.version = -1

    def ready(self, cell):
        if self.version != cell[0] or self.epoch != _PK_GLOBAL[0]:
            return False
        if self.stream != stream_ptr() and (self.captured or not lib._capturing()):
            torch.cuda.current_stream().wait_event(self.event)
        return True


def _stamp(st, built):
    ev = torch.cuda.Event()
    ev.record()
    cap = bool(lib._capturing())
    for im, cell in built:
        im.version, im.epoch, im.event, im.stream, im.captured = cell[0], _PK_GLOBAL[0], ev, st, cap


def _group_args(n, pointers, ints):
    VP, CI = ctypes.c_void_p * n, ctypes.c_int * n
    return [ctypes.cast(VP(*v), ctypes.c_void_p) for v in pointers] + [ctypes.cast(CI(*v), ctypes.c_void_p) for v in ints]


class WeightPacks:

    def __init__(self, w, version_cell=None):
        self.w = w
        self.cell = version_cell if version_cell is not None else [0]
        self.slots = {}
        self.elig = {}
        self.wino = {}
        self.wbytes = {}
        self.k4 = None
        self.k4pk = None

    def _pack(self, dgrad, slot):
        Cout, Cin, KH, KW = self.w.shape
        st = stream_ptr()
        stride, ph, pw = slot.geom
        call("mogan_pk_weight_pack", ptr(self.w), slot.buf.data_ptr(), Cout, Cin, KH, KW, stride, ph, pw, dgrad, st)
        _stamp(st, [(slot, self.cell)])
        PK_STATS["packs"] += 1

    def both_in_use(self):
        s0, s1 = self.slots.get(0), self.slots.get(1)
        Cout, Cin = self.w.shape[:2]
        return s0 is not None and s1 is not None and s0.geom == s1.geom and Cin % 32 == 0 and Cout % 32 == 0

    def adam_fusable(self):
        return self.both_in_use() and self.w.shape[2] * self.w.shape[3] in (16, 9, 1)

    def repack(self):
        s0, s1 = self.slots.get(0), self.slots.get(1)
        Cout, Cin, KH, KW = self.w.shape
        if self.both_in_use():
            stride, ph, pw = s0.geom
            st = stream_ptr()
            call("mogan_pk_weight_pack_both", ptr(self.w), s0.buf.data_ptr(), s1.buf.data_ptr(), Cout, Cin, KH, KW, stride, ph, pw, st)
            _stamp(st, [(s0, self.cell), (s1, self.cell)])
            PK_STATS["packs"] += 1
            return
        for dgrad, slot in self.slots.items():
            self._pack(dgrad, slot)

    def pointer(self, dgrad, B, Hs, Ws, stride, ph, pw):
        key = (dgrad, B, Hs, Ws, stride, ph, pw)
        e = self.elig.get(key)
        Cout, Cin, KH, KW = self.w.shape
        if e is None:
            e = self.elig[key] = bool(lib.load().mogan_pk_conv_eligible(B, Cin, Hs, Ws, Cout, KH, KW, stride, ph, pw, dgrad))
        if not e:
            return None
        slot = self.slots.get(dgrad)
        if slot is None:
            nbytes = int(lib.load().mogan_pk_weight_bytes(Cout, Cin, KH, KW, stride, dgrad))
            buf = torch.empty(nbytes, dtype=torch.uint8, device=self.w.device)
            slot = self.slots[dgrad] = WeightImage(buf, (stride, ph, pw))
        elif slot.geom != (stride, ph, pw):
            return None
        if not slot.ready(self.cell):
            self._pack(dgrad, slot)
        return slot.buf.data_ptr()

    def wino_pointer(self, dgrad, B, Hs, Ws, stride, ph, pw, up):
        key = (dgrad, B, Hs, Ws, stride, ph, pw, up)
        nb = self.wbytes.get(key)
        if nb is None:
            Cout, Cin, KH, KW = self.w.shape
            nb = self.wbytes[key] = int(lib.load().mogan_conv_prep_bytes(B, Cin, Hs, Ws, Cout, KH, KW, stride, ph, pw, up, dgrad))
        if not nb:
            return None
        im = self.wino.get(dgrad)
        if im is None or im.buf.numel() < nb:
            im = self.wino[dgrad] = WeightImage(torch.empty(nb, dtype=torch.uint8, device=self.w.device))
        if not im.ready(self.cell):
            wino_prep([(self, dgrad, im)])
        return im.buf.data_ptr()

    def k4_build(self):
        Cout, Cin = int(self.w.shape[0]), int(self.w.shape[1])
        st = stream_ptr()
        call("mogan_upconv3x3_k4", ptr(self.w), self.k4.buf.data_ptr(), Cout, Cin, st)
        _stamp(st, [(self.k4, self.cell)])
        PK_STATS["k4_builds"] = PK_STATS.get("k4_builds", 0) + 1

    def upconv_pointers(self, dgrad, B, Hs, Ws):
        if self.k4 is None:
            Cout, Cin = int(self.w.shape[0]), int(self.w.shape[1])
            self.k4 = WeightImage(torch.empty((Cin, Cout, 4, 4), dtype=torch.float32, device=self.w.device))
            self.k4pk = WeightPacks(self.k4.buf, self.cell)
        if not self.k4.ready(self.cell):
            self.k4_build()
        img = self.k4pk.wino_pointer(0 if dgrad else 1, B, 2 * Hs, 2 * Ws, 2, 1, 1, 0) if D2_PREP else None
        return self.k4.buf.data_ptr(), img

    def invalidate(self, version_cell):
        self.cell = version_cell
        for im in list(self.slots.values()) + list(self.wino.values()):
            im.invalidate()
        if self.k4 is not None:
            self.k4.invalidate()
            self.k4pk.invalidate(version_cell)


def wino_prep(items):
    n = len(items)
    if not n:
        return
    ws = [[pk.w.data_ptr() for pk, _, _ in items], [im.buf.data_ptr() for _, _, im in items]]
    shapes = [pk.w.shape for pk, _, _ in items]
    ints = [[s[i] for s in shapes] for i in (0, 1, 2)] + [[int(d) for _, d, _ in items]]
    st = stream_ptr()
    call("mogan_conv_prep_group", n, *_group_args(n, ws, ints), st)
    _stamp(st, [(im, pk.cell) for pk, _, im in items])
    PK_STATS["wino_preps"] = PK_STATS.get("wino_preps", 0) + 1


def k4_build_group(pks):
    n = len(pks)
    if not n:
        return
    ws = [[pk.w.data_ptr() for pk in pks], [pk.k4.buf.data_ptr() for pk in pks]]
    shapes = [pk.w.shape for pk in pks]
    st = stream_ptr()
    call("mogan_upconv3x3_k4_group", n, *_group_args(n, ws, [[s[i] for s in shapes] for i in (0, 1)]), st)
    _stamp(st, [(pk.k4, pk.cell) for pk in pks])
    PK_STATS["k4_builds"] = PK_STATS.get("k4_builds", 0) + 1


def repack_all(packs, packed=()):
    items, k4s = [], []
    for pk in packs:
        if id(pk) not in packed:
            pk.repack()
        items += [(pk, d, im) for d, im in pk.wino.items()]
        if pk.k4 is not None:
            k4s.append(pk)
            items += [(pk.k4pk, d, im) for d, im in pk.k4pk.wino.items()]
    k4_build_group(k4s)
    wino_prep(items)


def _wino_prep_ptr(w, dgrad, B, Hs, Ws, stride, ph, pw, up):
    pk = getattr(w, "_mogan_pk", None)
    if pk is None or not WINO_PREP:
        return None
    return pk.wino_pointer(dgrad, B, Hs, Ws, stride, ph, pw, up)


WINO_PREP = True


D2_PREP = True
UPCONV_OWNED = True


def _prep_kind(KH, KW, stride, up):
    return (KH == 3 and KW == 3 and stride == 1) or (D2_PREP and KH == 4 and KW == 4 and stride == 2 and not up)


def attach_packs(w, version_cell=None):
    pk = getattr(w, "_mogan_pk", None)
    if pk is None:
        pk = w._mogan_pk = WeightPacks(w, version_cell)
    elif version_cell is not None and pk.cell is not version_cell:
        pk.invalidate(version_cell)
    return pk


def _packed(w, dgrad, B, Hs, Ws, stride, ph, pw, up):
    if up or not PK_ENABLED:
        return None
    pk = getattr(w, "_mogan_pk", None)
    if pk is None:
        return None
    return pk.pointer(dgrad, B, Hs, Ws, stride, ph, pw)


def conv2d_forward(x, w, stride, ph, pw, up):
    B, Cin, Hs, Ws = x.shape
    Cout, _, KH, KW = w.shape
    wp = _packed(w, 0, B, Hs, Ws, stride, ph, pw, up)
    if wp is not None:
        OH, OW = conv_out_hw(Hs, Ws, KH, KW, stride, ph, pw, 0)
        y = torch.empty((B, Cout, OH, OW), dtype=torch.float32, device=x.device)
        wsp, wsn = workspace(x.device)
        call("mogan_conv2d_fwd_pk", ptr(x), wp, ptr(y), B, Cin, Hs, Ws, Cout, KH, KW, stride, ph, pw, wsp, wsn, stream_ptr())
        PK_STATS["fwd"] += 1
        return y
    if _is_upconv(w.shape, stride, ph, pw, up):
        y = torch.empty((B, Cout, 2 * Hs, 2 * Ws), dtype=torch.float32, device=x.device)
        wsp, wsn = workspace(x.device)
        pk = getattr(w, "_mogan_pk", None)
        if pk is not None and WINO_PREP and UPCONV_OWNED:
            k4, img = pk.upconv_pointers(0, B, Hs, Ws)
            call("mogan_conv2d_dgrad_wp", ptr(x), k4, img, ptr(y), B, Cout, 2 * Hs, 2 * Ws, Cin, 4, 4, 2, 1, 1, 0, wsp, wsn, stream_ptr())
            return y
        call("mogan_upconv3x3_fwd", ptr(x), ptr(w), ptr(y), B, Cin, Hs, Ws, Cout, wsp, wsn, stream_ptr())
        return y
    OH, OW = conv_out_hw(Hs, Ws, KH, KW, stride, ph, pw, up)
    y = torch.empty((B, Cout, OH, OW), dtype=torch.float32, device=x.device)
    wsp, wsn = workspace(x.device)
    wprep = _wino_prep_ptr(w, 0, B, Hs, Ws, stride, ph, pw, up) if _prep_kind(KH, KW, stride, up) else None
    if wprep is not None:
        call("mogan_conv2d_fwd_wp", ptr(x), ptr(w), wprep, ptr(y), B, Cin, Hs, Ws, Cout, KH, KW, stride, ph, pw, up,
             wsp, wsn, stream_ptr())
        return y
    call("mogan_conv2d_fwd", ptr(x), ptr(w), ptr(y), B, Cin, Hs, Ws, Cout, KH, KW, stride, ph, pw, up,
         wsp, wsn, stream_ptr())
    return y


def conv2d_dgrad(dy, w, x_shape, stride, ph, pw, up):
    B, Cin, Hs, Ws = x_shape
    Cout, _, KH, KW = w.shape
    wsp, wsn = workspace(dy.device)
    wp = _packed(w, 1, B, Hs, Ws, stride, ph, pw, up)
    if wp is not None:
        dx = torch.empty((B, Cin, Hs, Ws), dtype=torch.float32, device=dy.device)
        call("mogan_conv2d_dgrad_pk", ptr(dy), wp, ptr(dx), B, Cin, Hs, Ws, Cout, KH, KW, stride, ph, pw, wsp, wsn, stream_ptr())
        PK_STATS["dgrad"] += 1
        return dx
    if _is_upconv(w.shape, stride, ph, pw, up):
        dx = torch.empty((B, Cin, Hs, Ws), dtype=torch.float32, device=dy.device)
        pk = getattr(w, "_mogan_pk", None)
        if pk is not None and WINO_PREP and UPCONV_OWNED:
            k4, img = pk.upconv_pointers(1, B, Hs, Ws)
            call("mogan_conv2d_fwd_wp", ptr(dy), k4, img, ptr(dx), B, Cout, 2 * Hs, 2 * Ws, Cin, 4, 4, 2, 1, 1, 0, wsp, wsn, stream_ptr())
            return dx
        call("mogan_upconv3x3_dgrad", ptr(dy), ptr(w), ptr(dx), B, Cin, Hs, Ws, Cout, wsp, wsn, stream_ptr())
        return dx
    du = torch.empty((B, Cin, Hs << up, Ws << up), dtype=torch.float32, device=dy.device)
    wprep = _wino_prep_ptr(w, 1, B, Hs, Ws, stride, ph, pw, up) if _prep_kind(KH, KW, stride, up) else None
    if wprep is not None:
        call("mogan_conv2d_dgrad_wp", ptr(dy), ptr(w), wprep, ptr(du), B, Cin, Hs, Ws, Cout, KH, KW, stride, ph, pw, up,
             wsp, wsn, stream_ptr())
    else:
        call("mogan_conv2d_dgrad", ptr(dy), ptr(w), ptr(du), B, Cin, Hs, Ws, Cout, KH, KW, stride, ph, pw, up,
             wsp, wsn, stream_ptr())
    if not up:
        return du
    dx = torch.empty((B, Cin, Hs, Ws), dtype=torch.float32, device=dy.device)
    call("mogan_down2_sum", ptr(du), ptr(dx), B * Cin, Hs, Ws, stream_ptr())
    return dx


def conv2d_wgrad(dy, x, w_shape, stride, ph, pw, up, out=None, accumulate=False):
    B, Cin, Hs, Ws = x.shape
    Cout, _, KH, KW = w_shape
    wsp, wsn = workspace(dy.device)
    dw = out if out is not None else torch.empty(w_shape, dtype=torch.float32, device=dy.device)
    if PK_ENABLED and PK_WGRAD and not up:
        key = (B, Cin, Hs, Ws, Cout, KH, KW, stride, ph, pw, wsn)
        e = _pk_wgrad_elig.get(key)
        if e is None:
            e = _pk_wgrad_elig[key] = bool(lib.load().mogan_pk_wgrad_eligible(B, Cin, Hs, Ws, Cout, KH, KW, stride, ph, pw, wsn))
        if e:
            call("mogan_conv2d_wgrad_pk", ptr(dy), ptr(x), ptr(dw), B, Cin, Hs, Ws, Cout, KH, KW, stride, ph, pw,
                 1 if accumulate else 0, wsp, wsn, stream_ptr())
            PK_STATS["wgrad"] = PK_STATS.get("wgrad", 0) + 1
            return dw
    if _is_upconv(w_shape, stride, ph, pw, up):
        call("mogan_upconv3x3_wgrad", ptr(dy), ptr(x), ptr(dw), B, Cin, Hs, Ws, Cout, 1 if accumulate else 0, wsp, wsn,
             stream_ptr())
        return dw
    call("mogan_conv2d_wgrad", ptr(dy), ptr(x), ptr(dw), B, Cin, Hs, Ws, Cout, KH, KW, stride, ph, pw, up,
         1 if accumulate else 0, wsp, wsn, stream_ptr())
    return dw


class Conv2dFn(torch.autograd.Function):

    @staticmethod
    def forward(ctx, x, w, bias, stride, ph, pw, up):
        x, w = _c(x), _c(w)
        y = conv2d_forward(x, w, stride, ph, pw, up)
        if bias is not None:
            call("mogan_bias_add", ptr(y), ptr(_c(bias)), y.shape[0], y.shape[1], y.shape[2] * y.shape[3],
                 stream_ptr())
        ctx.save_for_backward(x, w)
        ctx.bias_ref = bias
        ctx.geom = (stride, ph, pw, up, bias is not None)
        return y

    @staticmethod
    def backward(ctx, dy):
        x, w = ctx.saved_tensors
        stride, ph, pw, up, has_bias = ctx.geom
        dy = _c(dy)
        dx = dw = db = None
        if ctx.needs_input_grad[0]:
            dx = conv2d_dgrad(dy, w, x.shape, stride, ph, pw, up)
        if ctx.needs_input_grad[1]:
            g = _grad_buf(w)
            if g is not None:
                _wgrad_accumulate(dy, x, w, (stride, ph, pw, up), g)
            else:
                dw = conv2d_wgrad(dy, x, w.shape, stride, ph, pw, up)
        if has_bias and ctx.needs_input_grad[2]:
            g = _grad_buf(ctx.bias_ref)
            db = g if g is not None else torch.empty(dy.shape[1], dtype=torch.float32, device=dy.device)
            call("mogan_bias_grad", ptr(dy), ptr(db), dy.shape[0], dy.shape[1], dy.shape[2] * dy.shape[3],
                 1 if g is not None else 0, stream_ptr())
            if g is not None:
                db = None
                _grad_hit(g)
        return dx, dw, db, None, None, None, None


class ConvAffineReluFn(torch.autograd.Function):

    @staticmethod
    def forward(ctx, x, w, scale, shift, stride, ph, pw):
        x, w = _c(x), _c(w)
        B, Cin, Hs, Ws = x.shape
        Cout, _, KH, KW = w.shape
        OH, OW = conv_out_hw(Hs, Ws, KH, KW, stride, ph, pw, 0)
        z = torch.empty((B, Cout, OH, OW), dtype=torch.float32, device=x.device)
        wsp, wsn = workspace(x.device)
        call("mogan_conv2d_affine_fwd", ptr(x), ptr(w), ptr(scale), ptr(shift), ptr(z), B, Cin, Hs, Ws, Cout, KH, KW,
             stride, ph, pw, 1, wsp, wsn, stream_ptr())
        ctx.save_for_backward(x, w, z, scale)
        ctx.geom = (stride, ph, pw)
        return z

    @staticmethod
    def backward(ctx, dz):
        x, w, z, scale = ctx.saved_tensors
        stride, ph, pw = ctx.geom
        dz = _c(dz)
        g = torch.empty_like(z)
        call("mogan_affine_relu_bwd_out", ptr(z), ptr(dz), ptr(scale), ptr(g), z.shape[0], z.shape[1],
             z.shape[2] * z.shape[3], stream_ptr())
        dx = conv2d_dgrad(g, w, x.shape, stride, ph, pw, 0) if ctx.needs_input_grad[0] else None
        dw = conv2d_wgrad(g, x, w.shape, stride, ph, pw, 0) if ctx.needs_input_grad[1] else None
        return dx, dw, None, None, None, None, None


class ConvLReLUFn(torch.autograd.Function):

    @staticmethod
    def forward(ctx, x, w, stride, ph, pw, slope):
        x, w = _c(x), _c(w)
        B, Cin, Hs, Ws = x.shape
        Cout, _, KH, KW = w.shape
        OH, OW = conv_out_hw(Hs, Ws, KH, KW, stride, ph, pw, 0)
        z = torch.empty((B, Cout, OH, OW), dtype=torch.float32, device=x.device)
        wsp, wsn = workspace(x.device)
        rc = lib.load().mogan_conv2d_lrelu_fwd(ptr(x), ptr(w), ptr(z), B, Cin, Hs, Ws, Cout, KH, KW, stride, ph, pw, slope,
                                               wsp, wsn, stream_ptr())
        if rc == 1:
            z = conv2d_forward(x, w, stride, ph, pw, 0)
            call("mogan_act_fwd", ptr(z), ptr(z), B, Cout, OH * OW, ACT_LRELU, slope, stream_ptr())
        elif rc != 0:
            raise lib.MoganHipError("mogan_conv2d_lrelu_fwd failed: %s" % lib._ERRORS.get(rc, rc))
        if ACT_TRACE is not None:
            _trace(ACT_LRELU, z, TRACE_GROUPS)
        ctx.save_for_backward(x, w, z)
        ctx.cfg = (stride, ph, pw, slope)
        return z

    @staticmethod
    def backward(ctx, dz):
        x, w, z = ctx.saved_tensors
        stride, ph, pw, slope = ctx.cfg
        g = torch.empty_like(z)
        call("mogan_act_bwd", ptr(z), ptr(_c(dz)), ptr(g), z.shape[0], z.shape[1], z.shape[2] * z.shape[3], ACT_LRELU, slope,
             stream_ptr())
        dx = conv2d_dgrad(g, w, x.shape, stride, ph, pw, 0) if ctx.needs_input_grad[0] else None
        dw = None
        if ctx.needs_input_grad[1]:
            gb = _grad_buf(w)
            if gb is not None:
                _wgrad_accumulate(g, x, w, (stride, ph, pw, 0), gb)
            else:
                dw = conv2d_wgrad(g, x, w.shape, stride, ph, pw, 0)
        return dx, dw, None, None, None, None


class LogitsHeadFn(torch.autograd.Function):

    @staticmethod
    def forward(ctx, x, w, bias):
        x, w = _c(x), _c(w)
        B, Cout, K = x.shape[0], w.shape[0], w[0].numel()
        p = torch.empty((B, Cout, 1, 1), dtype=torch.float32, device=x.device)
        call("mogan_logits_head_fwd", ptr(x), ptr(w), ptr(_c(bias)) if bias is not None else None, ptr(p), B, K, Cout,
             stream_ptr())
        ctx.save_for_backward(x, w, p)
        ctx.bias_ref = bias
        return p

    @staticmethod
    def backward(ctx, dp):
        x, w, p = ctx.saved_tensors
        bias = ctx.bias_ref
        B, Cout, K = x.shape[0], w.shape[0], w[0].numel()
        dp = _c(dp)
        dx = torch.empty_like(x) if ctx.needs_input_grad[0] else None
        want_w = ctx.needs_input_grad[1]
        want_b = bias is not None and ctx.needs_input_grad[2]
        gw = _grad_buf(w) if want_w else None
        gb = _grad_buf(bias) if want_b else None
        direct = (want_w or want_b) and (not want_w or gw is not None) and (not want_b or gb is not None)
        dw = gw if direct else (torch.empty_like(w) if want_w else None)
        db = (gb if direct else torch.empty_like(bias)) if want_b else None
        call("mogan_logits_head_bwd", ptr(dp), ptr(p), ptr(x), ptr(w), ptr(dx), ptr(dw), ptr(db), B, K, Cout,
             1 if direct else 0, stream_ptr())
        if direct:
            if gw is not None:
                _grad_hit(gw)
            if gb is not None:
                _grad_hit(gb)
            dw = db = None
        return dx, dw, db


def logits_head(x, w, bias):
    return LogitsHeadFn.apply(x, w, bias)


def logits_head_ok(x, conv):
    w = conv.weight
    ph, pw = conv.padding if isinstance(conv.padding, tuple) else (conv.padding, conv.padding)
    if not (x.dim() == 4 and ph == 0 and pw == 0 and w.shape[2] == x.shape[2] and w.shape[3] == x.shape[3] and w.shape[0] <= 4
            and w[0].numel() % 4 == 0 and x.shape[1] == w.shape[1]):
        return False
    return (not x.is_contiguous() or x.data_ptr() % 16 == 0) and (not w.is_contiguous() or w.data_ptr() % 16 == 0)


def conv2d_lrelu(x, w, stride, padding, slope=0.2):
    ph, pw = (padding, padding) if isinstance(padding, int) else padding
    return ConvLReLUFn.apply(x, w, int(stride), int(ph), int(pw), float(slope))


def conv2d_affine_relu(x, w, scale, shift, stride=1, padding=0):
    ph, pw = (padding, padding) if isinstance(padding, int) else padding
    return ConvAffineReluFn.apply(x, w, scale, shift, int(stride), int(ph), int(pw))


def conv2d(x, w, bias=None, stride=1, padding=0, up=False):
    ph, pw = (padding, padding) if isinstance(padding, int) else padding
    return Conv2dFn.apply(x, w, bias, int(stride), int(ph), int(pw), 1 if up else 0)


DEEP_STATS = {"fwd": 0, "bwd": 0, "panel_hits": 0}
DEEP_ENABLED = True
_deep_elig = {}


def pk_debug_force(take_all, cfg=-1, split=0):
    lib.load().mogan_pk_debug_force(int(take_all), int(cfg), int(split))
    _deep_elig.clear()
    _pk_wgrad_elig.clear()


def deep_block_eligible(x, w, stride, ph, pw, act, groups=1):
    if not (PK_ENABLED and DEEP_ENABLED) or getattr(w, "_mogan_pk", None) is None or x.dim() != 4:
        return False
    B, Cin, Hs, Ws = x.shape
    Cout, _, KH, KW = w.shape
    key = (B, Cin, Hs, Ws, Cout, KH, KW, stride, ph, pw, act, groups)
    e = _deep_elig.get(key)
    if e is None:
        e = _deep_elig[key] = bool(lib.load().mogan_deep_block_eligible(B, Cin, Hs, Ws, Cout, KH, KW, stride, ph, pw, act,
                                                                        groups))
    if e:
        pk = w._mogan_pk
        for d in (0, 1):
            slot = pk.slots.get(d)
            if slot is not None and slot.geom != (stride, ph, pw):
                return False
    return e


class DeepConvBNActFn(torch.autograd.Function):

    @staticmethod
    def forward(ctx, x, w, gamma, beta, running_mean, running_var, act, slope, eps, momentum, stride, ph, pw, groups):
        x, gamma, beta = _c(x), _c(gamma), _c(beta)
        B, Cin, Hs, Ws = x.shape
        Cout, _, KH, KW = w.shape
        OH, OW = conv_out_hw(Hs, Ws, KH, KW, stride, ph, pw, 0)
        dev = x.device
        pk = w._mogan_pk
        wp = pk.pointer(0, B, Hs, Ws, stride, ph, pw)
        if wp is None:
            raise lib.MoganHipError("deep block: no packed forward copy of this weight for geometry %r" % ((stride, ph, pw),))
        f32 = dict(dtype=torch.float32, device=dev)
        y = torch.empty((B, Cout, OH, OW), **f32)
        z = torch.empty((B, Cout, OH, OW), **f32)
        stats = torch.empty((2, groups, Cout), **f32)
        zpanel = torch.empty(int(lib.load().mogan_pk_panel_bytes(B, Cout, OH * OW)), dtype=torch.uint8, device=dev)
        xp = getattr(x, "_mogan_panel", None)
        if xp is not None and (xp[1] != x.data_ptr() or xp[2] != x._version):
            xp = None
        if xp is not None:
            DEEP_STATS["panel_hits"] += 1
        wsp, wsn = workspace(dev)
        if BN_DEFER is not None:
            if groups != 1:
                raise lib.MoganHipError("deferred running statistics: one BatchNorm call per launch only")
            BN_DEFER.append((stats[0, 0], stats[1, 0], B * OH * OW, running_mean, running_var, eps, momentum))
            running_mean = running_var = None
        call("mogan_deep_conv_bn_act_fwd", ptr(x), ptr(xp[0]) if xp is not None else None, wp, ptr(gamma), ptr(beta),
             ptr(running_mean), ptr(running_var), ptr(y), ptr(stats), ptr(z), ptr(zpanel), B, Cin, Hs, Ws, Cout, KH, KW,
             stride, ph, pw, eps, momentum, act, slope, groups, wsp, wsn, stream_ptr())
        DEEP_STATS["fwd"] += 1
        if ACT_TRACE is not None and act in (ACT_RELU, ACT_LRELU):
            _trace(act, z, groups)
        ctx.save_for_backward(x, w, y, stats, gamma, beta)
        ctx.cfg = (act, slope, stride, ph, pw, groups)
        z._mogan_panel = (zpanel, z.data_ptr(), z._version)
        return z

    @staticmethod
    def backward(ctx, dz):
        x, w, y, stats, gamma, beta = ctx.saved_tensors
        act, slope, stride, ph, pw, groups = ctx.cfg
        dz = _c(dz)
        B, Cin, Hs, Ws = x.shape
        Cout, _, KH, KW = w.shape
        dev = x.device
        dy = torch.empty_like(y)
        want_dx = ctx.needs_input_grad[0]
        dx = torch.empty(x.shape, dtype=torch.float32, device=dev) if want_dx else None
        wpd = w._mogan_pk.pointer(1, B, Hs, Ws, stride, ph, pw) if want_dx else None
        if want_dx and wpd is None:
            raise lib.MoganHipError("deep block: no packed data-gradient copy of this weight for geometry %r" % ((stride, ph, pw),))
        gg, gb = _grad_buf(gamma), _grad_buf(beta)
        want_gb = ctx.needs_input_grad[2] or ctx.needs_input_grad[3]
        direct = gg is not None and gb is not None and ctx.needs_input_grad[2] and ctx.needs_input_grad[3]
        dg = db = None
        if direct:
            pg, pb = gg, gb
        elif want_gb:
            dgb = torch.empty((2, Cout), dtype=torch.float32, device=dev)
            pg, pb = dgb[0], dgb[1]
        else:
            pg = pb = None
        wsp, wsn = workspace(dev)
        call("mogan_deep_conv_bn_act_bwd", ptr(dz), ptr(y), ptr(stats), ptr(gamma), ptr(beta), wpd, ptr(dy), ptr(pg), ptr(pb),
             1 if direct else 0, ptr(dx), B, Cin, Hs, Ws, Cout, KH, KW, stride, ph, pw, act, slope, groups, wsp, wsn,
             stream_ptr())
        DEEP_STATS["bwd"] += 1
        if direct:
            _grad_hit(gg)
            _grad_hit(gb)
        elif want_gb:
            dg, db = pg, pb
        dw = None
        if ctx.needs_input_grad[1]:
            g = _grad_buf(w)
            if g is not None:
                _wgrad_accumulate(dy, x, w, (stride, ph, pw, 0), g)
            else:
                dw = conv2d_wgrad(dy, x, w.shape, stride, ph, pw, 0)
        return (dx, dw, dg, db) + (None,) * 10


def deep_conv_bn_act(x, w, gamma, beta, running_mean, running_var, act, slope, eps, momentum, stride, ph, pw, groups=1):
    return DeepConvBNActFn.apply(x, w, gamma, beta, running_mean, running_var, int(act), float(slope), float(eps),
                                 float(momentum), int(stride), int(ph), int(pw), int(groups))


def bmm_raw(a, b, out, accumulate=False):
    Z_, M, K = a.shape
    N = b.shape[2]
    wsp, wsn = workspace(a.device)
    call("mogan_bmm", ptr(a), ptr(b), ptr(out), Z_, M, N, K,
         a.stride(0), a.stride(1), a.stride(2), b.stride(0), b.stride(1), b.stride(2),
         out.stride(0), out.stride(1), out.stride(2), 1 if accumulate else 0, wsp, wsn, stream_ptr())
    return out


class BmmFn(torch.autograd.Function):

    @staticmethod
    def forward(ctx, a, b):
        a, b = a.float(), b.float()
        out = torch.empty((a.shape[0], a.shape[1], b.shape[2]), dtype=torch.float32, device=a.device)
        bmm_raw(a, b, out)
        ctx.save_for_backward(a, b)
        return out

    @staticmethod
    def backward(ctx, dout):
        a, b = ctx.saved_tensors
        dout = _c(dout)
        da = db = None
        if ctx.needs_input_grad[0]:
            da = torch.empty(a.shape, dtype=torch.float32, device=a.device)
            bmm_raw(dout, b.transpose(1, 2), da)
        if ctx.needs_input_grad[1]:
            db = torch.empty(b.shape, dtype=torch.float32, device=a.device)
            bmm_raw(a.transpose(1, 2), dout, db)
        return da, db


def bmm(a, b):
    return BmmFn.apply(a, b)


class LinearFn(torch.autograd.Function):

    @staticmethod
    def forward(ctx, x, w, bias):
        x, w = _c(x), _c(w)
        y = torch.empty((x.shape[0], w.shape[0]), dtype=torch.float32, device=x.device)
        bmm_raw(x.unsqueeze(0), w.t().unsqueeze(0), y.unsqueeze(0))
        if bias is not None:
            call("mogan_bias_add", ptr(y), ptr(_c(bias)), y.shape[0], y.shape[1], 1, stream_ptr())
        ctx.save_for_backward(x, w)
        ctx.has_bias = bias is not None
        ctx.bias_ref = bias
        return y

    @staticmethod
    def backward(ctx, dy):
        x, w = ctx.saved_tensors
        dy = _c(dy)
        dx = dw = db = None
        if ctx.needs_input_grad[0]:
            dx = torch.empty(x.shape, dtype=torch.float32, device=x.device)
            bmm_raw(dy.unsqueeze(0), w.unsqueeze(0), dx.unsqueeze(0))
        if ctx.needs_input_grad[1]:
            g = _grad_buf(w)
            if g is not None:
                bmm_raw(dy.t().unsqueeze(0), x.unsqueeze(0), g.unsqueeze(0), accumulate=True)
                _grad_hit(g)
            else:
                dw = torch.empty(w.shape, dtype=torch.float32, device=x.device)
                bmm_raw(dy.t().unsqueeze(0), x.unsqueeze(0), dw.unsqueeze(0))
        if ctx.has_bias and ctx.needs_input_grad[2]:
            g = _grad_buf(ctx.bias_ref)
            db = g if g is not None else torch.empty(dy.shape[1], dtype=torch.float32, device=dy.device)
            call("mogan_bias_grad", ptr(dy), ptr(db), dy.shape[0], dy.shape[1], 1, 1 if g is not None else 0,
                 stream_ptr())
            if g is not None:
                db = None
                _grad_hit(g)
        return dx, dw, db


def linear(x, w, bias=None):
    return LinearFn.apply(x, w, bias)


def _bchw(x):
    if x.dim() == 2:
        return x.shape[0], x.shape[1], 1
    return x.shape[0], x.shape[1], x[0, 0].numel()


class BNActFn(torch.autograd.Function):

    @staticmethod
    def forward(ctx, x, gamma, beta, residual, running_mean, running_var, act, slope, eps, momentum, groups):
        x, gamma, beta = _c(x), _c(gamma), _c(beta)
        N, C, HW = _bchw(x)
        B = N // groups
        dev = x.device
        stats = torch.empty((2, groups, C), dtype=torch.float32, device=dev)
        Cy = C // 2 if act == ACT_GLU else C
        y = torch.empty((N, Cy) + tuple(x.shape[2:]), dtype=torch.float32, device=dev)
        one = bn_groups_ok(x, groups)
        if BN_DEFER is not None:
            if groups > 1:
                raise lib.MoganHipError("deferred running statistics: one BatchNorm call per launch only")
            BN_DEFER.append((stats[0, 0], stats[1, 0], B * HW, running_mean, running_var, eps, momentum))
            running_mean = running_var = None
        if one:
            call("mogan_bn_act_grouped_fwd", ptr(x), ptr(gamma), ptr(beta), ptr(running_mean), ptr(running_var), ptr(stats[0]),
                 ptr(stats[1]), ptr(y), groups, B, C, HW, act, slope, eps, momentum, stream_ptr())
        else:
            need = lib.bn_ws_bytes(B, C, HW)
            wsp, wsn = workspace(dev)
            if need > wsn:
                raise lib.MoganHipError("workspace too small for bn (%d > %d)" % (need, wsn))
            res = _c(residual) if residual is not None else None
            for g in range(groups):
                call("mogan_bn_act_fwd_fused", ptr(x[g * B:(g + 1) * B]), ptr(gamma), ptr(beta), ptr(res), ptr(running_mean),
                     ptr(running_var), ptr(stats[0, g]), ptr(stats[1, g]), ptr(y[g * B:(g + 1) * B]), B, C, HW, act, slope, eps,
                     momentum, wsp, wsn, stream_ptr())
        if ACT_TRACE is not None and act in (ACT_RELU, ACT_LRELU):
            _trace(act, y, groups)
        ctx.save_for_backward(x, gamma, beta, stats)
        ctx.cfg = (act, slope, groups, one, residual is not None)
        return y

    @staticmethod
    def backward(ctx, dy):
        x, gamma, beta, stats = ctx.saved_tensors
        act, slope, groups, one, has_res = ctx.cfg
        dy = _c(dy)
        N, C, HW = _bchw(x)
        B = N // groups
        dx = torch.empty_like(x)
        gg, gb = _grad_buf(gamma), _grad_buf(beta)
        direct = gg is not None and gb is not None and ctx.needs_input_grad[1] and ctx.needs_input_grad[2]
        loop_adds = groups > 1 and not one
        if direct:
            dg, db = gg, gb
        else:
            dgb = (torch.zeros if loop_adds else torch.empty)((2, C), dtype=torch.float32, device=x.device)
            dg, db = dgb[0], dgb[1]
        accumulate = 1 if direct or loop_adds else 0
        if one:
            call("mogan_bn_act_grouped_bwd", ptr(x), ptr(dy), ptr(stats[0]), ptr(stats[1]), ptr(gamma), ptr(beta), ptr(dx),
                 ptr(dg), ptr(db), groups, B, C, HW, act, slope, accumulate, stream_ptr())
        else:
            wsp, wsn = workspace(x.device)
            for g in range(groups):
                call("mogan_bn_act_bwd", ptr(x[g * B:(g + 1) * B]), ptr(dy[g * B:(g + 1) * B]), ptr(stats[0, g]), ptr(stats[1, g]),
                     ptr(gamma), ptr(beta), ptr(dx[g * B:(g + 1) * B]), ptr(dg), ptr(db), B, C, HW, act, slope, accumulate, wsp,
                     wsn, stream_ptr())
        if direct:
            _grad_hit(gg)
            _grad_hit(gb)
            dg = db = None
        return dx, dg, db, (dy if has_res else None), None, None, None, None, None, None, None


def bn_groups_ok(x, groups):
    N, C, HW = _bchw(x)
    return groups > 1 and N % groups == 0 and bool(lib.load().mogan_bn_act_grouped_eligible(groups, N // groups, C, HW))


def bn_act(x, gamma, beta, running_mean, running_var, act=ACT_NONE, slope=0.2, residual=None, eps=1e-5,
           momentum=0.1, groups=1):
    assert groups == 1 or residual is None
    return BNActFn.apply(x, gamma, beta, residual, running_mean, running_var, act, float(slope), float(eps), float(momentum),
                         int(groups))


class AffineActFn(torch.autograd.Function):

    @staticmethod
    def forward(ctx, x, scale, shift, act, slope):
        x = _c(x)
        B, C, HW = _bchw(x)
        y = torch.empty_like(x)
        call("mogan_affine_act_fwd", ptr(x), ptr(scale), ptr(shift), ptr(y), B, C, HW, act, slope, stream_ptr())
        ctx.save_for_backward(x, scale, shift)
        ctx.cfg = (act, slope)
        return y

    @staticmethod
    def backward(ctx, dy):
        x, scale, shift = ctx.saved_tensors
        act, slope = ctx.cfg
        B, C, HW = _bchw(x)
        dx = torch.empty_like(x)
        call("mogan_affine_act_bwd", ptr(x), ptr(_c(dy)), ptr(scale), ptr(shift), ptr(dx), B, C, HW, act, slope,
             stream_ptr())
        return dx, None, None, None, None


def affine_act(x, scale, shift, act=ACT_RELU, slope=0.0):
    return AffineActFn.apply(x, scale, shift, act, float(slope))


class ActFn(torch.autograd.Function):
    @staticmethod
    def forward(ctx, x, act, slope):
        x = _c(x)
        B, C, HW = _bchw(x)
        Cy = C // 2 if act == ACT_GLU else C
        y = torch.empty((B, Cy) + tuple(x.shape[2:]), dtype=torch.float32, device=x.device)
        call("mogan_act_fwd", ptr(x), ptr(y), B, C, HW, act, slope, stream_ptr())
        if ACT_TRACE is not None and act in (ACT_RELU, ACT_LRELU):
            ACT_TRACE.append((act, y))
        ctx.save_for_backward(x)
        ctx.cfg = (act, slope)
        return y

    @staticmethod
    def backward(ctx, dy):
        (x,) = ctx.saved_tensors
        act, slope = ctx.cfg
        B, C, HW = _bchw(x)
        dx = torch.empty_like(x)
        call("mogan_act_bwd", ptr(x), ptr(_c(dy)), ptr(dx), B, C, HW, act, slope, stream_ptr())
        return dx, None, None


def act(x, kind, slope=0.2):
    return ActFn.apply(x, kind, float(slope))


def glu(x):
    return ActFn.apply(x, ACT_GLU, 0.0)


class AddFn(torch.autograd.Function):
    @staticmethod
    def forward(ctx, a, b):
        a, b = _c(a), _c(b)
        y = torch.empty_like(a)
        call("mogan_add", ptr(a), ptr(b), ptr(y), a.numel(), stream_ptr())
        return y

    @staticmethod
    def backward(ctx, dy):
        return dy, dy


def add(a, b):
    return AddFn.apply(a, b)


class GroupSumFn(torch.autograd.Function):

    @staticmethod
    def forward(ctx, x, G):
        x = _c(x)
        y = torch.empty((x.shape[0] // G,) + tuple(x.shape[1:]), dtype=torch.float32, device=x.device)
        call("mogan_group_sum", ptr(x), ptr(y), y.numel(), G, stream_ptr())
        ctx.G = G
        return y

    @staticmethod
    def backward(ctx, dy):
        dy = _c(dy)
        dx = torch.empty((dy.shape[0] * ctx.G,) + tuple(dy.shape[1:]), dtype=torch.float32, device=dy.device)
        call("mogan_group_bcast", ptr(dy), ptr(dx), dy.numel(), ctx.G, stream_ptr())
        return dx, None


def group_sum(x, G):
    return GroupSumFn.apply(x, int(G))


class SoftmaxFn(torch.autograd.Function):

    @staticmethod
    def forward(ctx, x, dim, scale, lens):
        x = _c(x)
        dim = dim % x.dim()
        outer = 1
        for s in x.shape[:dim]:
            outer *= s
        inner = 1
        for s in x.shape[dim + 1:]:
            inner *= s
        L = x.shape[dim]
        y = torch.empty_like(x)
        call("mogan_softmax_fwd", ptr(x), ptr(y), ptr(lens), outer, L, inner, scale, stream_ptr())
        ctx.save_for_backward(y)
        ctx.lens = lens
        ctx.cfg = (outer, L, inner, scale)
        return y

    @staticmethod
    def backward(ctx, dy):
        (y,) = ctx.saved_tensors
        outer, L, inner, scale = ctx.cfg
        dx = torch.empty_like(y)
# ... 1247 lines not shown
```

Baseline: 458.8.

## Compute deep-block weight gradients directly from packed bf16x3 panels

Adds a panel-based wgrad kernel that consumes the already-packed split-bf16 x panel from forward and a dY panel written by the fused BN/activation backward tail, instead of re-packing fp32 dy and x inside the wgrad GEMM. It also handles merged wgrad batches as multiple segments, so the two pending batches no longer have to be concatenated with torch.cat. The cost is extra memory for persistent x panels (packed in forward when none exists) and dY panels, plus an allow-list of layer shapes that restricts where the path is used.

```diff
diff --git a/include/mogan_hip.h b/include/mogan_hip.h
--- a/include/mogan_hip.h
+++ b/include/mogan_hip.h
@@ -121,6 +121,19 @@
                                const void* wpk_dgrad, float* dy, float* dgamma, float* dbeta, int accumulate, float* dx, int B,
                                int Cin, int Hs, int Ws, int Cout, int KH, int KW, int stride, int ph, int pw, int act, float slope,
                                int groups, void* ws, size_t ws_bytes, hipStream_t stream);
+int mogan_deep_conv_bn_act_bwd_panel(const float* dz, const float* y, const float* stats, const float* gamma, const float* beta,
+                                     const void* wpk_dgrad, float* dy, void* dypanel, float* dgamma, float* dbeta, int accumulate,
+                                     float* dx, int B, int Cin, int Hs, int Ws, int Cout, int KH, int KW, int stride, int ph, int pw,
+                                     int act, float slope, int groups, void* ws, size_t ws_bytes, hipStream_t stream);
+
+int mogan_pk_panel_pack(const float* x, void* panel, int B, int C, int HW, hipStream_t stream);
+
+typedef struct MoganPanelSeg { const void* x; const void* dy; int B; } MoganPanelSeg;
+int mogan_conv2d_wgrad_panels_eligible(int B, int Cin, int Hs, int Ws, int Cout, int KH, int KW, int stride, int ph, int pw);
+size_t mogan_conv2d_wgrad_panels_ws(int nseg, const MoganPanelSeg* segs, int Cin, int Hs, int Ws, int Cout, int KH, int KW, int stride,
+                                    int ph, int pw, hipStream_t stream);
+int mogan_conv2d_wgrad_panels(int nseg, const MoganPanelSeg* segs, float* dw, int Cin, int Hs, int Ws, int Cout, int KH, int KW,
+                              int stride, int ph, int pw, int accumulate, void* ws, size_t ws_bytes, hipStream_t stream);
 
 typedef struct MoganPkArgs {
     const void* wpk; const void* panel; float* raw;
diff --git a/multiple-objects-gan_amd/csrc/mogan_internal.h b/multiple-objects-gan_amd/csrc/mogan_internal.h
--- a/multiple-objects-gan_amd/csrc/mogan_internal.h
+++ b/multiple-objects-gan_amd/csrc/mogan_internal.h
@@ -33,6 +33,7 @@
 MOGAN_HIDDEN int mogan_stem_fwd_try(const float* x, const float* w, float* y, const MoganConvShape& g, float slope, hipStream_t st);
 MOGAN_HIDDEN int mogan_dconv2_prep_group(int n, const float* const* w, void* const* prep, const int* Cout, const int* Cin,
                                          const int* dgrad, hipStream_t st);
+MOGAN_HIDDEN void mogan_pk_forced(int* take_all, int* cfg, int* split);
 MOGAN_HIDDEN void mogan_prof_begin(int mode, int cfg, double flops, int M, int N, int K, hipStream_t st);
 MOGAN_HIDDEN void mogan_prof_end(int taken, hipStream_t st);
 MOGAN_HIDDEN void mogan_prof_relabel(int cfg);
diff --git a/multiple-objects-gan_amd/csrc/mogan_pgemm.hip b/multiple-objects-gan_amd/csrc/mogan_pgemm.hip
--- a/multiple-objects-gan_amd/csrc/mogan_pgemm.hip
+++ b/multiple-objects-gan_amd/csrc/mogan_pgemm.hip
@@ -780,11 +780,20 @@
 
 }
 
+void mogan_pk_forced(int* take_all, int* cfg, int* split) { *take_all = g_pk_force; *cfg = g_pk_cfg; *split = g_pk_split; }
+
 extern "C" {
 
 int mogan_pk_debug_force(int take_all, int cfg, int split) {
     g_pk_force = take_all; g_pk_cfg = (cfg >= 0 && cfg < NPK) ? cfg : -1; g_pk_split = split > 0 ? split : 0;
     return 0;
+}
+
+int mogan_pk_panel_pack(const float* x, void* panel, int B, int C, int HW, hipStream_t stream) {
+    if (!x || !panel || ((uintptr_t)panel & 15) != 0 || B <= 0 || C <= 0 || C % 32 || HW <= 0) return MOGAN_ERR_SHAPE;
+    if ((unsigned long long)B * HW * C * 6ull >= (1ull << 32) || C / 32 > 65535) return MOGAN_ERR_SHAPE;
+    apack(x, (unsigned char*)panel, B, C, HW, stream);
+    return hipGetLastError() == hipSuccess ? 0 : MOGAN_ERR_LAUNCH;
 }
 
 int mogan_pk_conv_eligible(int B, int Cin, int Hs, int Ws, int Cout, int KH, int KW, int stride, int ph, int pw, int dgrad) {
@@ -1081,10 +1090,12 @@
     return hipGetLastError() == hipSuccess ? 0 : MOGAN_ERR_LAUNCH;
 }
 
-int mogan_deep_conv_bn_act_bwd(const float* dz, const float* y, const float* stats, const float* gamma, const float* beta,
-                               const void* wpk_dgrad, float* dy, float* dgamma, float* dbeta, int accumulate, float* dx, int B,
-                               int Cin, int Hs, int Ws, int Cout, int KH, int KW, int stride, int ph, int pw, int act, float slope,
-                               int groups, void* ws, size_t ws_bytes, hipStream_t stream) {
+}
+
+static int deep_bwd(const float* dz, const float* y, const float* stats, const float* gamma, const float* beta,
+                    const void* wpk_dgrad, float* dy, void* dypanel, float* dgamma, float* dbeta, int accumulate, float* dx, int B,
+                    int Cin, int Hs, int Ws, int Cout, int KH, int KW, int stride, int ph, int pw, int act, float slope,
+                    int groups, void* ws, size_t ws_bytes, hipStream_t stream) {
     if (B <= 0 || stride <= 0 || groups < 1 || B % groups || Cin % 32 || KH <= 0 || KW <= 0 || KH * KW > 25) return MOGAN_ERR_SHAPE;
     const int OH = (Hs + 2 * ph - KH) / stride + 1, OW = (Ws + 2 * pw - KW) / stride + 1;
     if (OH <= 0 || OW <= 0 || !tail_ok(B / groups, Cout, OH * OW, act, groups) || !dz || !y || !stats || !gamma || !beta || !dy)
@@ -1092,17 +1103,39 @@
     const size_t pbytes = up256((size_t)B * OH * OW * Cout * 6);
     const bool want_dx = dx != nullptr;
     if (want_dx && !deep_geom_ok(B, Cin, Hs, Ws, Cout, KH, KW, stride, OH, OW, 1)) return MOGAN_ERR_SHAPE;
-    if (want_dx && (!ws || ws_bytes < pbytes || !wpk_dgrad)) return MOGAN_ERR_WS;
+    if (dypanel && ((uintptr_t)dypanel & 15) != 0) return MOGAN_ERR_SHAPE;
+    if (want_dx && ((!dypanel && (!ws || ws_bytes < pbytes)) || !wpk_dgrad)) return MOGAN_ERR_WS;
+    unsigned char* panel = dypanel ? (unsigned char*)dypanel : want_dx ? (unsigned char*)ws : nullptr;
+    const size_t wused = dypanel ? 0 : pbytes;
     TailBwdP t{};
     t.dz = dz; t.y = y; t.mean = stats; t.invstd = stats + (size_t)groups * Cout; t.gamma = gamma; t.beta = beta; t.dy = dy;
-    t.dypanel = want_dx ? (unsigned char*)ws : nullptr; t.dgamma = dgamma; t.dbeta = dbeta; t.accumulate = accumulate;
+    t.dypanel = panel; t.dgamma = dgamma; t.dbeta = dbeta; t.accumulate = accumulate;
     t.B = B / groups; t.G = groups; t.C = Cout; t.HW = OH * OW; t.slope = slope;
     if (act == MOGAN_ACT_LRELU) launch_tail_bwd<MOGAN_ACT_LRELU>(t, stream);
     else if (act == MOGAN_ACT_RELU) launch_tail_bwd<MOGAN_ACT_RELU>(t, stream);
     else launch_tail_bwd<MOGAN_ACT_NONE>(t, stream);
     if (!want_dx) return hipGetLastError() == hipSuccess ? 0 : MOGAN_ERR_LAUNCH;
-    return pk_dgrad_from_panel(ws, wpk_dgrad, dx, B, Cin, Hs, Ws, Cout, KH, KW, stride, ph, pw, (char*)ws + pbytes,
-                               ws_bytes - pbytes, stream);
-}
-
-}
+    return pk_dgrad_from_panel(panel, wpk_dgrad, dx, B, Cin, Hs, Ws, Cout, KH, KW, stride, ph, pw, ws ? (char*)ws + wused : nullptr,
+                               ws ? ws_bytes - wused : 0, stream);
+}
+
+extern "C" {
+
+int mogan_deep_conv_bn_act_bwd(const float* dz, const float* y, const float* stats, const float* gamma, const float* beta,
+                               const void* wpk_dgrad, float* dy, float* dgamma, float* dbeta, int accumulate, float* dx, int B,
+                               int Cin, int Hs, int Ws, int Cout, int KH, int KW, int stride, int ph, int pw, int act, float slope,
+                               int groups, void* ws, size_t ws_bytes, hipStream_t stream) {
+    return deep_bwd(dz, y, stats, gamma, beta, wpk_dgrad, dy, nullptr, dgamma, dbeta, accumulate, dx, B, Cin, Hs, Ws, Cout, KH, KW,
+                    stride, ph, pw, act, slope, groups, ws, ws_bytes, stream);
+}
+
+int mogan_deep_conv_bn_act_bwd_panel(const float* dz, const float* y, const float* stats, const float* gamma, const float* beta,
+                                     const void* wpk_dgrad, float* dy, void* dypanel, float* dgamma, float* dbeta, int accumulate,
+                                     float* dx, int B, int Cin, int Hs, int Ws, int Cout, int KH, int KW, int stride, int ph, int pw,
+                                     int act, float slope, int groups, void* ws, size_t ws_bytes, hipStream_t stream) {
+    if (!dypanel) return MOGAN_ERR_SHAPE;
+    return deep_bwd(dz, y, stats, gamma, beta, wpk_dgrad, dy, dypanel, dgamma, dbeta, accumulate, dx, B, Cin, Hs, Ws, Cout, KH, KW,
+                    stride, ph, pw, act, slope, groups, ws, ws_bytes, stream);
+}
+
+}
diff --git a/multiple-objects-gan_amd/csrc/mogan_pwgrad.hip b/multiple-objects-gan_amd/csrc/mogan_pwgrad.hip
--- /dev/null
+++ b/multiple-objects-gan_amd/csrc/mogan_pwgrad.hip
@@ -0,0 +1,341 @@
+#include <hip/hip_runtime.h>
+#include <stdint.h>
+#include <algorithm>
+#include "../../include/mogan_hip.h"
+#include "mogan_internal.h"
+#include "mogan_mma.h"
+
+namespace {
+
+typedef short pw_s16x4 __attribute__((ext_vector_type(4)));
+typedef short pw_s16x8 __attribute__((ext_vector_type(8)));
+typedef __attribute__((address_space(3))) pw_s16x4 pw_lds_s16x4;
+
+constexpr int PW_MAXSEG = 4;
+constexpr int PW_KT = 16;
+constexpr int PW_UNIT = PW_KT * 192;
+
+struct PwP {
+    const unsigned char* x[PW_MAXSEG]; const unsigned char* dy[PW_MAXSEG];
+    unsigned xbytes[PW_MAXSEG], dybytes[PW_MAXSEG];
+    int npix[PW_MAXSEG], tend[PW_MAXSEG];
+    int nseg;
+    float* C; float* ws;
+    int M, CGy, CGx, U, R;
+    int KHW, KW, Hs, Ws, OW, OHW, s, ph, pw;
+    unsigned mOHW, mOW;
+    int ntile, kt_per, nsplit;
+    long long slab;
+    int accumulate;
+    int gx, gy;
+};
+
+__device__ __forceinline__ unsigned pw_div(unsigned n, unsigned d, unsigned m) { return d == 1 ? n : __umulhi(n, m); }
+
+__device__ __forceinline__ uint4 pw_ldg16(__amdgpu_buffer_rsrc_t r, unsigned off, bool ok) {
+    return __builtin_bit_cast(uint4, __builtin_amdgcn_raw_buffer_load_b128(r, ok ? off : 0xFFFFFFF0u, 0, 0));
+}
+
+__device__ __forceinline__ mma_bf16x8 pw_tr_frag(const unsigned char* lds) {
+    const pw_s16x4 lo = __builtin_amdgcn_ds_read_tr16_b64_v4i16((pw_lds_s16x4*)(lds));
+    const pw_s16x4 hi = __builtin_amdgcn_ds_read_tr16_b64_v4i16((pw_lds_s16x4*)(lds + 4 * 192));
+    const pw_s16x8 v = __builtin_shufflevector(lo, hi, 0, 1, 2, 3, 4, 5, 6, 7);
+    return __builtin_bit_cast(mma_bf16x8, v);
+}
+
+template <int TM, int TN, int WM>
+__device__ __forceinline__ void pwgrad_body(const PwP& p) {
+    constexpr int WN = 4 / WM;
+    constexpr int BM = WM * TM * 32, BN = WN * TN * 32, UA = BM / 32, UB = BN / 32;
+    constexpr int BUF = (UA + UB) * PW_UNIT;
+    constexpr int NA = UA * 12 / 16, NB = (UB * 12 + 15) / 16;
+    static_assert(UA * 12 % 16 == 0, "whole chunk rounds of the dY tile");
+    constexpr int EU = UB == 4 ? 40 : 48, EP = UB * EU;
+    static_assert(32 * EP * 4 <= 2 * BUF, "the epilogue image fits the staging buffers");
+    __shared__ __attribute__((aligned(16))) unsigned char Ls[2 * BUF];
+
+    const int tid = threadIdx.x, lane = tid & 63, wave = tid >> 6;
+    const int wm = wave % WM, wn = wave / WM;
+    unsigned V = mma_xcd_order(blockIdx.x, gridDim.x);
+    const unsigned bx = V % p.gx; V /= p.gx;
+    const unsigned by = V % p.gy;
+    const int sp = V / p.gy;
+    const int t_beg = sp * p.kt_per, t_end = min(p.ntile, t_beg + p.kt_per);
+
+    const int k = tid >> 4, sub = tid & 15;
+    unsigned offA[NA], ldsA[NA]; bool okA[NA];
+#pragma unroll
+    for (int i = 0; i < NA; ++i) {
+        const int j = sub + 16 * i, ua = j / 12, ch = j - ua * 12;
+        const int cg = by * UA + ua;
+        okA[i] = cg < p.CGy;
+        offA[i] = (unsigned)cg * 192u + ch * 16;
+        ldsA[i] = ua * PW_UNIT + k * 192 + ch * 16;
+    }
+    unsigned offB[NB], ldsB[NB]; int dyB[NB], dxB[NB]; bool okB[NB];
+#pragma unroll
+    for (int i = 0; i < NB; ++i) {
+        int j = sub + 16 * i;
+        if (j >= UB * 12) j -= 16;
+        const int ub = j / 12, ch = j - ub * 12;
+        const int u = bx * UB + ub;
+        okB[i] = u < p.U;
+        const int uu = okB[i] ? u : 0;
+        const int cg = uu / p.KHW, tap = uu - cg * p.KHW, kh = tap / p.KW, kw = tap - kh * p.KW;
+        dyB[i] = kh - p.ph; dxB[i] = kw - p.pw;
+        offB[i] = (unsigned)cg * 192u + ch * 16;
+        ldsB[i] = (UA + ub) * PW_UNIT + k * 192 + ch * 16;
+    }
+    const unsigned pixA = (unsigned)p.CGy * 192u, pixB = (unsigned)p.CGx * 192u;
+
+    mma_f32x16 acc[TM][TN];
+#pragma unroll
+    for (int a = 0; a < TM; ++a)
+#pragma unroll
+        for (int b = 0; b < TN; ++b)
+#pragma unroll
+            for (int r = 0; r < 16; ++r) acc[a][b][r] = 0.f;
+
+    uint4 ra[NA], rb[NB];
+    auto load = [&](int t) {
+        const unsigned char* xs = p.x[0]; const unsigned char* ys = p.dy[0];
+        unsigned xb = p.xbytes[0], yb = p.dybytes[0];
+        int np = p.npix[0], t0 = 0;
+#pragma unroll
+        for (int i = 1; i < PW_MAXSEG; ++i)
+            if (i < p.nseg && t >= p.tend[i - 1]) { xs = p.x[i]; ys = p.dy[i]; xb = p.xbytes[i]; yb = p.dybytes[i]; np = p.npix[i]; t0 = p.tend[i - 1]; }
+        const __amdgpu_buffer_rsrc_t rX = __builtin_amdgcn_make_buffer_rsrc((void*)xs, (short)0, (int)xb, 0x00020000);
+        const __amdgpu_buffer_rsrc_t rY = __builtin_amdgcn_make_buffer_rsrc((void*)ys, (short)0, (int)yb, 0x00020000);
+        const int n = (t - t0) * PW_KT + k;
+        const bool live = (int)(t < t_end) & (int)(n < np);
+        const unsigned nn = live ? (unsigned)n : 0u;
+#pragma unroll
+        for (int i = 0; i < NA; ++i) {
+            unsigned off = nn * pixA + offA[i];
+            asm volatile("" : "+v"(off));
+            ra[i] = pw_ldg16(rY, off, (int)live & (int)okA[i]);
+        }
+        const unsigned img = pw_div(nn, p.OHW, p.mOHW), rem = nn - img * p.OHW;
+        const unsigned oy = pw_div(rem, p.OW, p.mOW), ox = rem - oy * p.OW;
+        const int iy0 = (int)oy * p.s, ix0 = (int)ox * p.s;
+        const unsigned pb = img * (unsigned)(p.Hs * p.Ws);
+#pragma unroll
+        for (int i = 0; i < NB; ++i) {
+            const int iy = iy0 + dyB[i], ix = ix0 + dxB[i];
+            const bool ok = (int)live & (int)okB[i] & (int)((unsigned)iy < (unsigned)p.Hs) & (int)((unsigned)ix < (unsigned)p.Ws);
+            unsigned off = (pb + (unsigned)(iy * p.Ws + ix)) * pixB + offB[i];
+            asm volatile("" : "+v"(off));
+            rb[i] = pw_ldg16(rX, off, ok);
+        }
+    };
+    auto store = [&](int buf) {
+#pragma unroll
+        for (int i = 0; i < NA; ++i) *(uint4*)(&Ls[buf * BUF + ldsA[i]]) = ra[i];
+#pragma unroll
+        for (int i = 0; i < NB; ++i) *(uint4*)(&Ls[buf * BUF + ldsB[i]]) = rb[i];
+    };
+    const int g = lane >> 4, q = (lane >> 2) & 3, pp = lane & 3;
+    const int troff = (8 * (g >> 1) + q) * 192 + (16 * (g & 1) + 4 * pp) * 2;
+    auto compute = [&](int buf) {
+        const unsigned char* base = &Ls[buf * BUF + troff];
+        X6Frag fa[TM];
+#pragma unroll
+        for (int ta = 0; ta < TM; ++ta)
+#pragma unroll
+            for (int pl = 0; pl < 3; ++pl) fa[ta].p[pl] = pw_tr_frag(base + (wm * TM + ta) * PW_UNIT + pl * 64);
+#pragma unroll
+        for (int tb = 0; tb < TN; ++tb) {
+            X6Frag fb;
+#pragma unroll
+            for (int pl = 0; pl < 3; ++pl) fb.p[pl] = pw_tr_frag(base + (UA + wn * TN + tb) * PW_UNIT + pl * 64);
+#pragma unroll
+            for (int term = 0; term < 6; ++term)
+#pragma unroll
+                for (int ta = 0; ta < TM; ++ta) acc[ta][tb] = x6_mfma(fa[ta], fb, term, acc[ta][tb]);
+        }
+    };
+
+    load(t_beg);
+    store(0);
+    __syncthreads();
+    for (int t = t_beg; t < t_end; t += 2) {
+        load(t + 1);
+        compute(0);
+        store(1);
+        __syncthreads();
+        load(t + 2);
+        compute(1);
+        store(0);
+        __syncthreads();
+    }
+
+    const bool split = p.nsplit > 1;
+    float* __restrict__ out = split ? p.ws + (size_t)sp * p.slab : p.C;
+    const bool addc = !split && p.accumulate;
+    float* E = (float*)Ls;
+    const int ub = tid % UB;
+    const int u = bx * UB + ub;
+    const bool uok = u < p.U;
+    const int uu = uok ? u : 0;
+    const int ecg = uu / p.KHW, etap = uu - ecg * p.KHW;
+    const size_t colbase = (size_t)ecg * 32 * p.KHW + etap;
+#pragma unroll
+    for (int wmi = 0; wmi < WM; ++wmi) {
+#pragma unroll
+        for (int ta = 0; ta < TM; ++ta) {
+            if (wm == wmi) {
+#pragma unroll
+                for (int tb = 0; tb < TN; ++tb)
+#pragma unroll
+                    for (int r16 = 0; r16 < 16; ++r16) {
+                        const int row = (r16 & 3) + 8 * (r16 >> 2) + 4 * (lane >> 5);
+                        E[row * EP + (wn * TN + tb) * EU + (lane & 31)] = acc[ta][tb][r16];
+                    }
+            }
+            __syncthreads();
+            const int row0 = by * BM + (wmi * TM + ta) * 32;
+#pragma unroll
+            for (int it = 0; it < 4 * UB; ++it) {
+                const int idx = it * 256 + tid;
+                const int ci = (idx / UB) & 31, row = idx / (UB * 32);
+                const int m = row0 + row;
+                if (uok && m < p.M) {
+                    float v = E[row * EP + ub * EU + ci];
+                    float* dst = out + (size_t)m * p.R + colbase + (size_t)ci * p.KHW;
+                    if (addc) v += *dst;
+                    *dst = v;
+                }
+            }
+            __syncthreads();
+        }
+    }
+}
+
+template <int TM, int TN, int WM, int OCC>
+__global__ __launch_bounds__(256, OCC) void pwgrad_kernel(const PwP p) { pwgrad_body<TM, TN, WM>(p); }
+
+static inline long long cdiv(long long a, long long b) { return (a + b - 1) / b; }
+static inline unsigned magic(unsigned d) { return d <= 1 ? 0u : 0xFFFFFFFFu / d + 1u; }
+
+struct PwCfg { int bm, bn; };
+static const PwCfg kPw[3] = {{128, 128}, {128, 64}, {256, 64}};
+
+struct PwGeom { int OH, OW, KHW; long long R, numel; };
+
+static bool pw_geom(int Cin, int Hs, int Ws, int Cout, int KH, int KW, int stride, int ph, int pw, PwGeom& g) {
+    if (Cin <= 0 || Cout <= 0 || Cin % 32 || Cout % 32 || Hs <= 0 || Ws <= 0 || KH <= 0 || KW <= 0 || stride <= 0 || ph < 0 || pw < 0)
+        return false;
+    if ((long long)KH * KW > 25) return false;
+    g.KHW = KH * KW;
+    g.OH = (Hs + 2 * ph - KH) / stride + 1; g.OW = (Ws + 2 * pw - KW) / stride + 1;
+    if (Hs + 2 * ph < KH || Ws + 2 * pw < KW || g.OH <= 0 || g.OW <= 0) return false;
+    if ((long long)g.OH * g.OW > 4096 || (long long)Hs * Ws > (1 << 20)) return false;
+    g.R = (long long)Cin * g.KHW; g.numel = (long long)Cout * g.R;
+    return g.numel < (1ll << 31);
+}
+
+static bool pw_seg(int B, int Cin, int Hs, int Ws, int Cout, const PwGeom& g, long long& npix, unsigned long long& xb, unsigned long long& yb) {
+    if (B <= 0) return false;
+    npix = (long long)B * g.OH * g.OW;
+    xb = (unsigned long long)B * Hs * Ws * Cin * 6ull; yb = (unsigned long long)npix * Cout * 6ull;
+    return npix <= (1 << 20) && xb < (1ull << 32) && yb < (1ull << 32);
+}
+
+struct PwPlan { int cfg, gx, gy, kt_per, nsplit; };
+
+static PwPlan pw_plan(int Cout, long long U, int ntile, hipStream_t st) {
+    int take_all = 0, fcfg = -1, fsplit = 0;
+    mogan_pk_forced(&take_all, &fcfg, &fsplit);
+    PwPlan pl{};
+    const int target = mogan_split_target(st);
+    auto tiles_of = [&](int c) { return cdiv(Cout, kPw[c].bm) * cdiv(U * 32, kPw[c].bn); };
+    int best = (tiles_of(0) < target && tiles_of(1) >= target) ? 1 : 0;
+    if (fcfg >= 0 && fcfg < 3) best = fcfg;
+    pl.cfg = best;
+    pl.gx = (int)cdiv(U * 32, kPw[best].bn); pl.gy = (int)cdiv(Cout, kPw[best].bm);
+    const long long tiles = (long long)pl.gx * pl.gy;
+    int nsplit = 1;
+    if (tiles < target && ntile >= 8) {
+        nsplit = (int)cdiv(target, tiles);
+        nsplit = std::min(nsplit, ntile / 4);
+        if (nsplit < 1) nsplit = 1;
+    }
+    if (fsplit > 0) nsplit = std::min(fsplit, ntile);
+    pl.kt_per = (int)cdiv(cdiv(ntile, nsplit), 2) * 2;
+    pl.nsplit = (int)cdiv(ntile, pl.kt_per);
+    return pl;
+}
+
+static int pw_ntile(int nseg, const MoganPanelSeg* segs, const PwGeom& g) {
+    long long nt = 0;
+    for (int i = 0; i < nseg; ++i) nt += cdiv((long long)segs[i].B * g.OH * g.OW, PW_KT);
+    return (int)nt;
+}
+
+}
+
+extern "C" {
+
+int mogan_conv2d_wgrad_panels_eligible(int B, int Cin, int Hs, int Ws, int Cout, int KH, int KW, int stride, int ph, int pw) {
+    PwGeom g; long long npix; unsigned long long xb, yb;
+    if (!pw_geom(Cin, Hs, Ws, Cout, KH, KW, stride, ph, pw, g) || !pw_seg(B, Cin, Hs, Ws, Cout, g, npix, xb, yb)) return 0;
+    int take_all = 0, fcfg = -1, fsplit = 0;
+    mogan_pk_forced(&take_all, &fcfg, &fsplit);
+    if (take_all) return 1;
+    return g.OH * g.OW <= 256 && npix >= 128 && Cout >= 128 && g.R >= 1024;
+}
+
+size_t mogan_conv2d_wgrad_panels_ws(int nseg, const MoganPanelSeg* segs, int Cin, int Hs, int Ws, int Cout, int KH, int KW, int stride,
+                                    int ph, int pw, hipStream_t stream) {
+    PwGeom g;
+    if (!segs || nseg < 1 || nseg > PW_MAXSEG || !pw_geom(Cin, Hs, Ws, Cout, KH, KW, stride, ph, pw, g)) return 0;
+    for (int i = 0; i < nseg; ++i) {
+        long long npix; unsigned long long xb, yb;
+        if (!pw_seg(segs[i].B, Cin, Hs, Ws, Cout, g, npix, xb, yb)) return 0;
+    }
+    const PwPlan pl = pw_plan(Cout, (long long)(Cin / 32) * g.KHW, pw_ntile(nseg, segs, g), stream);
+    return pl.nsplit > 1 ? (size_t)pl.nsplit * (size_t)g.numel * sizeof(float) : 0;
+}
+
+int mogan_conv2d_wgrad_panels(int nseg, const MoganPanelSeg* segs, float* dw, int Cin, int Hs, int Ws, int Cout, int KH, int KW,
+                              int stride, int ph, int pw, int accumulate, void* ws, size_t ws_bytes, hipStream_t stream) {
+    PwGeom g;
+    if (!segs || nseg < 1 || nseg > PW_MAXSEG || !dw || ((uintptr_t)dw & 15) != 0) return MOGAN_ERR_SHAPE;
+    if (!pw_geom(Cin, Hs, Ws, Cout, KH, KW, stride, ph, pw, g)) return MOGAN_ERR_SHAPE;
+    PwP p{};
+    long long nt = 0;
+    for (int i = 0; i < nseg; ++i) {
+        long long npix; unsigned long long xb, yb;
+        if (!segs[i].x || !segs[i].dy || (((uintptr_t)segs[i].x | (uintptr_t)segs[i].dy) & 15) != 0) return MOGAN_ERR_SHAPE;
+        if (!pw_seg(segs[i].B, Cin, Hs, Ws, Cout, g, npix, xb, yb)) return MOGAN_ERR_SHAPE;
+        nt += cdiv(npix, PW_KT);
+        p.x[i] = (const unsigned char*)segs[i].x; p.dy[i] = (const unsigned char*)segs[i].dy;
+        p.xbytes[i] = (unsigned)xb; p.dybytes[i] = (unsigned)yb; p.npix[i] = (int)npix; p.tend[i] = (int)nt;
+    }
+    for (int i = nseg; i < PW_MAXSEG; ++i) { p.x[i] = p.x[0]; p.dy[i] = p.dy[0]; p.tend[i] = (int)nt; }
+    const long long U = (long long)(Cin / 32) * g.KHW;
+    const PwPlan pl = pw_plan(Cout, U, (int)nt, stream);
+    const size_t need = pl.nsplit > 1 ? (size_t)pl.nsplit * (size_t)g.numel * sizeof(float) : 0;
+    if (need && (!ws || ((uintptr_t)ws & 15) != 0 || ws_bytes < need)) return MOGAN_ERR_WS;
+    const long long blocks = (long long)pl.gx * pl.gy * pl.nsplit;
+    if (blocks <= 0 || blocks > 0x7fffffff) return MOGAN_ERR_SHAPE;
+    p.nseg = nseg; p.C = dw; p.ws = (float*)ws;
+    p.M = Cout; p.CGy = Cout / 32; p.CGx = Cin / 32; p.U = (int)U; p.R = (int)g.R;
+    p.KHW = g.KHW; p.KW = KW; p.Hs = Hs; p.Ws = Ws; p.OW = g.OW; p.OHW = g.OH * g.OW; p.s = stride; p.ph = ph; p.pw = pw;
+    p.mOHW = magic((unsigned)p.OHW); p.mOW = magic((unsigned)p.OW);
+    p.ntile = (int)nt; p.kt_per = pl.kt_per; p.nsplit = pl.nsplit; p.slab = g.numel; p.accumulate = accumulate ? 1 : 0;
+    p.gx = pl.gx; p.gy = pl.gy;
+    double K = 0;
+    for (int i = 0; i < nseg; ++i) K += (double)p.npix[i];
+    mogan_prof_begin(9, pl.cfg, 2.0 * (double)g.numel * K, Cout, (int)g.R, (int)K, stream);
+    switch (pl.cfg) {
+        case 1: hipLaunchKernelGGL((pwgrad_kernel<1, 2, 4, 3>), dim3((unsigned)blocks), dim3(256), 0, stream, p); break;
+        case 2: hipLaunchKernelGGL((pwgrad_kernel<2, 2, 4, 2>), dim3((unsigned)blocks), dim3(256), 0, stream, p); break;
+        default: hipLaunchKernelGGL((pwgrad_kernel<2, 2, 2, 2>), dim3((unsigned)blocks), dim3(256), 0, stream, p); break;
+    }
+    mogan_prof_end(1, stream);
+    if (pl.nsplit > 1) mogan_splitk_reduce_dense((const float*)ws, dw, g.numel, pl.nsplit, p.accumulate, stream);
+    return hipGetLastError() == hipSuccess ? 0 : MOGAN_ERR_LAUNCH;
+}
+
+}
diff --git a/multiple-objects-gan_amd/hip/lib.py b/multiple-objects-gan_amd/hip/lib.py
--- a/multiple-objects-gan_amd/hip/lib.py
+++ b/multiple-objects-gan_amd/hip/lib.py
@@ -51,6 +51,11 @@
     "mogan_deep_block_eligible": [I] * 12,
     "mogan_deep_conv_bn_act_fwd": [P] * 11 + [I] * 10 + [F, F, I, F, I, P, Z, P],
     "mogan_deep_conv_bn_act_bwd": [P] * 9 + [I, P] + [I] * 10 + [I, F, I, P, Z, P],
+    "mogan_deep_conv_bn_act_bwd_panel": [P] * 10 + [I, P] + [I] * 10 + [I, F, I, P, Z, P],
+    "mogan_pk_panel_pack": [P, P, I, I, I, P],
+    "mogan_conv2d_wgrad_panels_eligible": [I] * 10,
+    "mogan_conv2d_wgrad_panels_ws": [I, P] + [I] * 9 + [P],
+    "mogan_conv2d_wgrad_panels": [I, P, P] + [I] * 10 + [P, Z, P],
     "mogan_upconv3x3_ws_bytes": [I, I],
     "mogan_upconv3x3_fwd": [P, P, P, I, I, I, I, I, P, Z, P],
     "mogan_lstm_encoder_fwd": [P] * 11 + [I] * 6 + [P],
@@ -187,6 +192,10 @@
                                                                        "KH", "KW", "stride", "ph", "pw", "dgrad", "nsplit")]
 
 
+class PanelSeg(ctypes.Structure):
+    _fields_ = [("x", P), ("dy", P), ("B", I)]
+
+
 class TailArgs(ctypes.Structure):
     _fields_ = [("src", P * 3), ("src_bs", L * 3), ("src_slab", L * 3), ("src_nsplit", I * 3), ("nsrc", I), ("add", P), ("add_bs", L),
                 ("mask", P), ("mask_bs", L), ("scale", P), ("shift", P), ("relu", I), ("box", I), ("dst", P), ("dst_bs", L),
@@ -197,7 +206,7 @@
             "mogan_wino_prep_bytes": Z, "mogan_conv_prep_bytes": Z, "mogan_poly3_mmd_ws_bytes": Z,
             "mogan_knn_sqdist_ws_bytes": Z, "mogan_ball_count_ws_bytes": Z, "mogan_swd_moments_ws_bytes": Z,
             "mogan_ssim_level_ws_bytes": Z, "mogan_knn_cross_ws_bytes": Z, "mogan_radial_power_ws_bytes": Z,
-            "mogan_knn_label_ws_bytes": Z, "mogan_softmax_head_ws_bytes": Z}
+            "mogan_knn_label_ws_bytes": Z, "mogan_softmax_head_ws_bytes": Z, "mogan_conv2d_wgrad_panels_ws": Z}
 _ERRORS = {-1: "MOGAN_ERR_SHAPE", -2: "MOGAN_ERR_LAUNCH", -3: "MOGAN_ERR_WS"}
 
 _lib = None
diff --git a/multiple-objects-gan_amd/hip/ops.py b/multiple-objects-gan_amd/hip/ops.py
--- a/multiple-objects-gan_amd/hip/ops.py
+++ b/multiple-objects-gan_amd/hip/ops.py
@@ -115,43 +115,59 @@
     return first
 
 
-def _wgrad_launch(dy, x, w_shape, geom, g):
+def _wgrad_launch(dy, x, w_shape, geom, g, panels=None, prev=None):
     stride, ph, pw, up = geom
+    segs = None
+    if PANEL_WGRAD and panels is not None and not up and (prev is None or prev[2] is not None):
+        segs = ([(prev[2][0], prev[2][1], prev[0].shape[0])] if prev is not None else []) + [(panels[0], panels[1], dy.shape[0])]
+        if not panel_wgrad_eligible(sum(s[2] for s in segs), x.shape, w_shape, stride, ph, pw, [s[2] for s in segs]):
+            segs = None
+    if segs is None and prev is not None:
+        dy, x = _cat_batch(prev[0], dy), _cat_batch(prev[1], x)
     acc = not _first_of_round(g)
+
+    def run():
+        if segs is not None and conv2d_wgrad_panels(segs, x.shape, w_shape, stride, ph, pw, g, acc):
+            return
+        if segs is not None and prev is not None:
+            conv2d_wgrad(_cat_batch(prev[0], dy), _cat_batch(prev[1], x), w_shape, stride, ph, pw, up, out=g, accumulate=acc)
+        else:
+            conv2d_wgrad(dy, x, w_shape, stride, ph, pw, up, out=g, accumulate=acc)
+
     if WGRAD_SIDE_STREAM:
         cur, side = _wgrad_stream()
         side.wait_stream(cur)
         with torch.cuda.stream(side):
-            conv2d_wgrad(dy, x, w_shape, stride, ph, pw, up, out=g, accumulate=acc)
+            run()
         fr = _wgrad_frames[-1]
         if side not in fr.used:
             fr.used.append(side)
-        fr.keep.append((dy, x))
+        fr.keep.append((dy, x, panels, prev))
         _grad_hit(g, side)
     else:
-        conv2d_wgrad(dy, x, w_shape, stride, ph, pw, up, out=g, accumulate=acc)
+        run()
         _grad_hit(g)
 
 
-def _wgrad_accumulate(dy, x, w, geom, g):
+def _wgrad_accumulate(dy, x, w, geom, g, panels=None):
     K = dy.shape[0] * dy.shape[2] * dy.shape[3]
     if not (MERGE_WGRAD and _wgrad_ctx_depth > 0 and K <= _MERGE_K and w.numel() >= _MERGE_W) \
             or (torch.cuda.is_current_stream_capturing() and not MERGE_WGRAD_CAPTURED):
-        _wgrad_launch(dy, x, w.shape, geom, g)
+        _wgrad_launch(dy, x, w.shape, geom, g, panels)
         return
     cur = torch.cuda.current_stream()
     key = (g.data_ptr(), cur.cuda_stream)
     prev = _wgrad_pending.pop(key, None)
     if prev is None:
-        _wgrad_pending[key] = (dy, x, tuple(w.shape), geom, g, cur)
+        _wgrad_pending[key] = (dy, x, tuple(w.shape), geom, g, cur, panels)
         _wgrad_frames[-1].parked.append(key)
         return
     pdy, px, _, pgeom = prev[:4]
     if pgeom == geom and pdy.shape[1:] == dy.shape[1:] and px.shape[1:] == x.shape[1:]:
-        _wgrad_launch(_cat_batch(pdy, dy), _cat_batch(px, x), w.shape, geom, g)
+        _wgrad_launch(dy, x, w.shape, geom, g, panels, prev=(pdy, px, prev[6]))
     else:
-        _wgrad_launch(pdy, px, w.shape, pgeom, g)
-        _wgrad_launch(dy, x, w.shape, geom, g)
+        _wgrad_launch(pdy, px, w.shape, pgeom, g, prev[6])
+        _wgrad_launch(dy, x, w.shape, geom, g, panels)
 
 
 def _cat_batch(a, b):
@@ -197,12 +213,12 @@
         item = _wgrad_pending.pop(key, None)
         if item is None:
             continue
-        dy, x, w_shape, geom, g, st = item
+        dy, x, w_shape, geom, g, st, panels = item
         if st.cuda_stream == cur.cuda_stream:
-            _wgrad_launch(dy, x, w_shape, geom, g)
+            _wgrad_launch(dy, x, w_shape, geom, g, panels)
         else:
             with torch.cuda.stream(st):
-                _wgrad_launch(dy, x, w_shape, geom, g)
+                _wgrad_launch(dy, x, w_shape, geom, g, panels)
             if not capturing:
                 cur.wait_stream(st)
 
@@ -588,6 +604,58 @@
     return dw
 
 
+PANEL_WGRAD = os.environ.get("MOGAN_PANEL_WGRAD", "1") != "0"
+PANEL_WGRAD_LAYERS = {(1536, 3072, 4, 2, 16), (768, 1536, 4, 2, 64), (3072, 1536, 3, 1, 16), (768, 1536, 4, 2, 16)}
+PANEL_WGRAD_STATS = {"launches": 0, "segments": 0, "declined_ws": 0}
+_panel_wgrad_elig = {}
+_pk_take_all = [False]
+
+
+def panel_wgrad_eligible(B, x_shape, w_shape, stride, ph, pw, segments=None):
+    _, Cin, Hs, Ws = x_shape
+    Cout, _, KH, KW = w_shape
+    key = (B, Cin, Hs, Ws, Cout, KH, KW, stride, ph, pw)
+    e = _panel_wgrad_elig.get(key)
+    if e is None:
+        e = _panel_wgrad_elig[key] = bool(lib.load().mogan_conv2d_wgrad_panels_eligible(*key))
+    if not e or _pk_take_all[0]:
+        return e
+    OH, OW = conv_out_hw(Hs, Ws, KH, KW, stride, ph, pw, 0)
+    if PANEL_WGRAD_LAYERS is not None and (Cin, Cout, KH, stride, OH * OW) not in PANEL_WGRAD_LAYERS:
+        return False
+    if segments is None:
+        return True
+    if any((b * OH * OW) % 16 for b in segments[:-1]):
+        return False
+    if not (PK_ENABLED and PK_WGRAD):
+        return False
+    pk = key + (lib.WORKSPACE_BYTES,)
+    e = _pk_wgrad_elig.get(pk)
+    if e is None:
+        e = _pk_wgrad_elig[pk] = bool(lib.load().mogan_pk_wgrad_eligible(*pk))
+    return e
+
+
+def conv2d_wgrad_panels(segs, x_shape, w_shape, stride, ph, pw, out, accumulate):
+    _, Cin, Hs, Ws = x_shape
+    Cout, _, KH, KW = w_shape
+    arr = (lib.PanelSeg * len(segs))()
+    for i, (xp, dyp, b) in enumerate(segs):
+        arr[i].x, arr[i].dy, arr[i].B = ptr(xp), ptr(dyp), int(b)
+    ap = ctypes.cast(arr, ctypes.c_void_p)
+    wsp, wsn = workspace(out.device)
+    st = stream_ptr()
+    if int(lib.load().mogan_conv2d_wgrad_panels_ws(len(segs), ap, Cin, Hs, Ws, Cout, KH, KW, stride, ph, pw, st)) > wsn:
+        PANEL_WGRAD_STATS["declined_ws"] += 1
+        return False
+    call("mogan_conv2d_wgrad_panels", len(segs), ap, ptr(out), Cin, Hs, Ws, Cout, KH, KW, stride, ph, pw, 1 if accumulate else 0,
+         wsp, wsn, st)
+    PK_STATS["wgrad"] = PK_STATS.get("wgrad", 0) + 1
+    PANEL_WGRAD_STATS["launches"] += 1
+    PANEL_WGRAD_STATS["segments"] += len(segs)
+    return True
+
+
 class Conv2dFn(torch.autograd.Function):
 
     @staticmethod
@@ -772,6 +840,8 @@
     lib.load().mogan_pk_debug_force(int(take_all), int(cfg), int(split))
     _deep_elig.clear()
     _pk_wgrad_elig.clear()
+    _panel_wgrad_elig.clear()
+    _pk_take_all[0] = bool(take_all)
 
 
 def deep_block_eligible(x, w, stride, ph, pw, act, groups=1):
@@ -816,6 +886,12 @@
             xp = None
         if xp is not None:
             DEEP_STATS["panel_hits"] += 1
+        keep = PANEL_WGRAD and w.requires_grad and panel_wgrad_eligible(B, x.shape, w.shape, stride, ph, pw)
+        if keep and xp is None:
+            own = torch.empty(int(lib.load().mogan_pk_panel_bytes(B, Cin, Hs * Ws)), dtype=torch.uint8, device=dev)
+            call("mogan_pk_panel_pack", ptr(x), ptr(own), B, Cin, Hs * Ws, stream_ptr())
+            xp = (own, x.data_ptr(), x._version)
+        ctx.xpanel = xp[0] if keep else None
         wsp, wsn = workspace(dev)
         if BN_DEFER is not None:
             if groups != 1:
@@ -859,9 +935,17 @@
         else:
             pg = pb = None
         wsp, wsn = workspace(dev)
-        call("mogan_deep_conv_bn_act_bwd", ptr(dz), ptr(y), ptr(stats), ptr(gamma), ptr(beta), wpd, ptr(dy), ptr(pg), ptr(pb),
-             1 if direct else 0, ptr(dx), B, Cin, Hs, Ws, Cout, KH, KW, stride, ph, pw, act, slope, groups, wsp, wsn,
-             stream_ptr())
+        g = _grad_buf(w) if ctx.needs_input_grad[1] else None
+        dypanel = None
+        if PANEL_WGRAD and g is not None and ctx.xpanel is not None:
+            dypanel = torch.empty(int(lib.load().mogan_pk_panel_bytes(B, Cout, y.shape[2] * y.shape[3])), dtype=torch.uint8, device=dev)
+            call("mogan_deep_conv_bn_act_bwd_panel", ptr(dz), ptr(y), ptr(stats), ptr(gamma), ptr(beta), wpd, ptr(dy), ptr(dypanel),
+                 ptr(pg), ptr(pb), 1 if direct else 0, ptr(dx), B, Cin, Hs, Ws, Cout, KH, KW, stride, ph, pw, act, slope, groups,
+                 wsp, wsn, stream_ptr())
+        else:
+            call("mogan_deep_conv_bn_act_bwd", ptr(dz), ptr(y), ptr(stats), ptr(gamma), ptr(beta), wpd, ptr(dy), ptr(pg), ptr(pb),
+                 1 if direct else 0, ptr(dx), B, Cin, Hs, Ws, Cout, KH, KW, stride, ph, pw, act, slope, groups, wsp, wsn,
+                 stream_ptr())
         DEEP_STATS["bwd"] += 1
         if direct:
             _grad_hit(gg)
@@ -870,9 +954,8 @@
             dg, db = pg, pb
         dw = None
         if ctx.needs_input_grad[1]:
-            g = _grad_buf(w)
             if g is not None:
-                _wgrad_accumulate(dy, x, w, (stride, ph, pw, 0), g)
+                _wgrad_accumulate(dy, x, w, (stride, ph, pw, 0), g, (ctx.xpanel, dypanel) if dypanel is not None else None)
             else:
                 dw = conv2d_wgrad(dy, x, w.shape, stride, ph, pw, 0)
         return (dx, dw, dg, db) + (None,) * 10
```

Result: no change. 457.8 (-0.2%).
